# BVE-Reborn/rend3

Hardware: AMD Instinct MI355X
Metric: shaded Mpixels/s @4K (whole frame: cull+compact all cameras, 4 shadow views, PBR opaque, tonemap) (higher is better)
Workload: dtype f32; 1 GPU; BASELINE.json configs[2] stand-in: bistro_like (seed 0xB157, every object owns its geometry), 3840x2160, full PBR opaque + 4 directional shadow views (2048^2), camera dolly, 130 materials with base colour + normal + AO/roughness/metallic maps (RGBA8, mips, trilinear); objects=3000, triangles=2823212, cameras=5, parallelism=single GPU

## Files before the change

bindings/rend3-amd-sys/src/lib.rs:

```rust
#![allow(non_camel_case_types, non_upper_case_globals, clippy::too_many_arguments)]
use std::os::raw::{c_char, c_int, c_void};

pub const R3N_OK: i32 = 0;
pub const R3N_ERR_INVALID_ARG: i32 = -1;
pub const R3N_ERR_HIP: i32 = -2;
pub const R3N_ERR_NO_DEVICE: i32 = -3;
pub const R3N_ERR_STATE: i32 = -4;
pub const R3N_ERR_UNSUPPORTED: i32 = -5;
pub const R3N_ERR_CAPACITY: i32 = -6;
pub const R3N_CAMERA_VIEWPORT: u32 = 0xFFFFFFFF;
pub const R3N_MAX_SHADOW_VIEWS: u32 = 64;
pub const R3N_PASS_DEPTH: u32 = 0;
pub const R3N_PASS_FORWARD: u32 = 1;
pub const R3N_SOURCE_PREDICTED: u32 = 0;
pub const R3N_SOURCE_RESIDUAL: u32 = 1;
pub const R3N_KEY_OPAQUE: u32 = 0;
pub const R3N_KEY_CUTOUT: u32 = 1;
pub const R3N_KEY_BLEND: u32 = 2;
pub const R3N_TEXTURE_RGBA8_UNORM: u32 = 0;
pub const R3N_TEXTURE_RGBA8_UNORM_SRGB: u32 = 1;
pub const R3N_TEXTURE_R8_UNORM: u32 = 2;
pub const R3N_TEXTURE_RG8_UNORM: u32 = 3;
pub const R3N_TEXTURE_BGRA8_UNORM: u32 = 4;
pub const R3N_TEXTURE_BGRA8_UNORM_SRGB: u32 = 5;
// ... 374 lines not shown
}

#[repr(C)]
#[derive(Clone, Copy)]
pub struct r3n_texture_tail_result {
    pub textures: u64,
    pub words_copied: u64,
    pub kernel_launches: u64,
    pub full_syncs: u64,
    pub pool_words_after: u64,
}

#[repr(C)]
#[derive(Clone, Copy)]
pub struct r3n_texture_counters {
    pub update_calls: u64,
    pub kernel_launches: u64,
    pub bytes_staged: u64,
    pub full_syncs: u64,
    pub pool_grows: u64,
    pub pool_words: u64,
    pub live_words: u64,
    pub free_ranges: u64,
}

#[repr(C)]
#[derive(Clone, Copy)]
pub struct r3n_sample_query40 {
    pub id: [u32; 3],
    pub nearest: u32,
    pub u: f32,
    pub v: f32,
    pub ddx: [f32; 2],
    pub ddy: [f32; 2],
}

#[repr(C)]
#[derive(Clone, Copy)]
pub struct r3n_sample_result52 {
    pub rgba: [[f32; 4]; 3],
    pub flags: u32,
}

#[repr(C)]
#[derive(Clone, Copy)]
pub struct r3n_shadow_view272 {
    pub header: r3n_camera_header240,
    pub x: u32,
    pub y: u32,
    pub size: u32,
    pub _pad: [u32; 5],
}

#[repr(C)]
#[derive(Clone, Copy)]
pub struct r3n_frame_desc {
    pub struct_size: u32,
    pub flags: u32,
    pub width: u32,
    pub height: u32,
    pub samples: u32,
    pub shadow_atlas_width: u32,
    pub shadow_atlas_height: u32,
    pub n_shadow_views: u32,
    pub clear_color: [f32; 4],
    pub uniforms: *const r3n_frame_uniforms496,
    pub viewport_header: *const r3n_camera_header240,
    pub shadow_views: *const r3n_shadow_view272,
    pub shadow_view_mask: u64,
    pub directional_buffer: *const c_void,
    pub directional_bytes: u64,
    pub point_buffer: *const c_void,
    pub point_bytes: u64,
    pub skin_inputs: *const r3n_skinning_input40,
    pub n_skeletons: u32,
    pub n_joint_matrices: u32,
    pub joint_matrices: *const f32,
    pub exchange: r3n_exchange_fn,
    pub exchange_user: *mut c_void,
}

#[repr(C)]
#[derive(Clone, Copy)]
pub struct r3n_tri_ref {
    pub object: u32,
    pub triangle: u32,
}

#[repr(C)]
#[derive(Clone, Copy)]
pub struct r3n_host_camera144 {
    pub view: [f32; 16],
    pub projection_kind: u32,
    pub handedness: u32,
    pub aspect_ratio: f32,
    pub _pad: u32,
    pub projection_params: [f32; 16],
}

#[repr(C)]
#[derive(Clone, Copy)]
pub struct r3n_host_directional_light48 {
    pub color: [f32; 3],
    pub intensity: f32,
    pub direction: [f32; 3],
    pub distance: f32,
    pub resolution: u32,
    pub _pad: [u32; 3],
}

#[repr(C)]
#[derive(Clone, Copy)]
pub struct r3n_host_frame {
    pub uniforms: r3n_frame_uniforms496,
    pub viewport_header: r3n_camera_header240,
    pub shadow_atlas_width: u32,
    pub shadow_atlas_height: u32,
    pub n_shadow_views: u32,
    pub _pad0: u32,
    pub camera_location: [f32; 3],
    pub _pad1: f32,
    pub view_proj: [f32; 16],
    pub shadow_views: [r3n_shadow_view272; R3N_MAX_SHADOW_VIEWS as usize],
    pub shadow_handles: [u32; R3N_MAX_SHADOW_VIEWS as usize],
    pub directional_bytes: u64,
    pub directional_buffer: [u8; 8208],
}

#[link(name = "rend3_amd")]
extern "C" {
    pub fn r3n_create(hip_device: c_int, config: *const r3n_config) -> *mut r3n_ctx;
    pub fn r3n_destroy(ctx: *mut r3n_ctx);
    pub fn r3n_last_error(ctx: *const r3n_ctx) -> *const c_char;
    pub fn r3n_create_error() -> *const c_char;
    pub fn r3n_sync(ctx: *mut r3n_ctx) -> c_int;
    pub fn r3n_stream(ctx: *mut r3n_ctx) -> *mut c_void;
    pub fn r3n_mesh_buffer_write(ctx: *mut r3n_ctx, byte_offset: u64, data: *const c_void, bytes: u64) -> c_int;
    pub fn r3n_mesh_blocks_add(ctx: *mut r3n_ctx, blocks: *const r3n_mesh_block24, n: u32, payload: *const c_void, payload_bytes: u64, byte_offsets_out: *mut u64) -> c_int;
    pub fn r3n_mesh_blocks_remove(ctx: *mut r3n_ctx, byte_offsets: *const u64, n: u32) -> c_int;
    pub fn r3n_mesh_compact(ctx: *mut r3n_ctx, opts: *const r3n_mesh_compact_opts, result: *mut r3n_mesh_compact_result, moves_out: *mut r3n_mesh_move24, moves_capacity: u32) -> c_int;
    pub fn r3n_mesh_stats(ctx: *mut r3n_ctx, out: *mut r3n_mesh_counters, reset: c_int) -> c_int;
    pub fn r3n_objects_write(ctx: *mut r3n_ctx, slots: *const u32, records: *const r3n_object128, n: u32, capacity: u32) -> c_int;
    pub fn r3n_materials_write(ctx: *mut r3n_ctx, slots: *const u32, records: *const r3n_material208, keys: *const u8, n: u32) -> c_int;
    pub fn r3n_textures_write(ctx: *mut r3n_ctx, descs: *const r3n_texture_desc32, n_textures: u32, texels: *const u32, n_texels: u64) -> c_int;
    pub fn r3n_textures_write_encoded(ctx: *mut r3n_ctx, descs: *const r3n_texture_desc32, n_textures: u32, payload: *const c_void, payload_bytes: u64) -> c_int;
    pub fn r3n_textures_update(ctx: *mut r3n_ctx, slots: *const u32, descs: *const r3n_texture_desc32, n: u32, payload: *const c_void, payload_bytes: u64) -> c_int;
    pub fn r3n_textures_remove(ctx: *mut r3n_ctx, slots: *const u32, n: u32) -> c_int;
    pub fn r3n_textures_compact(ctx: *mut r3n_ctx, opts: *const r3n_texture_compact_opts, out: *mut r3n_texture_compact_result) -> c_int;
    pub fn r3n_textures_from_texture(ctx: *mut r3n_ctx, items: *const r3n_texture_tail16, n: u32, out: *mut r3n_texture_tail_result) -> c_int;
    pub fn r3n_texture_stats(ctx: *mut r3n_ctx, out: *mut r3n_texture_counters, reset: c_int) -> c_int;
    pub fn r3n_sample_probe(ctx: *mut r3n_ctx, form: u32, queries: *const r3n_sample_query40, n: u32, out: *mut r3n_sample_result52) -> c_int;
    pub fn r3n_texture_cubes_write(ctx: *mut r3n_ctx, descs: *const r3n_texture_desc32, n_cubes: u32, texels: *const u32, n_texels: u64) -> c_int;
    pub fn r3n_skybox_set(ctx: *mut r3n_ctx, cube_id: u32) -> c_int;
    pub fn r3n_blend_order_write(ctx: *mut r3n_ctx, objects_back_to_front: *const u32, n: u32) -> c_int;
    pub fn r3n_blend_objects_write(ctx: *mut r3n_ctx, slots: *const u32, locations: *const f32, n: u32) -> c_int;
    pub fn r3n_blend_sort(ctx: *mut r3n_ctx, camera_location: *const f32) -> c_int;
    pub fn r3n_lights_write(ctx: *mut r3n_ctx, directional_buffer: *const c_void, directional_bytes: u64, point_buffer: *const c_void, point_bytes: u64) -> c_int;
    pub fn r3n_set_output_format(ctx: *mut r3n_ctx, format: u32) -> c_int;
    pub fn r3n_set_skinning_mode(ctx: *mut r3n_ctx, mode: u32) -> c_int;
    pub fn r3n_set_shade_mode(ctx: *mut r3n_ctx, mode: u32) -> c_int;
    pub fn r3n_frame_begin(ctx: *mut r3n_ctx, uniforms: *const r3n_frame_uniforms496, width: u32, height: u32, samples: u32, clear_color: *const f32, shadow_atlas_width: u32, shadow_atlas_height: u32) -> c_int;
    pub fn r3n_skinning(ctx: *mut r3n_ctx, inputs: *const r3n_skinning_input40, n_skeletons: u32, joint_matrices: *const f32, n_joint_matrices: u32) -> c_int;
    pub fn r3n_animation_write(ctx: *mut r3n_ctx, rigs: *const r3n_anim_rig16, n_rigs: u32, joints: *const r3n_anim_joint80, n_joints: u32, clips: *const r3n_anim_clip16, n_clips: u32, tracks: *const r3n_anim_track80, n_tracks: u32, times: *const f32, n_times: u32, values: *const f32, n_values: u32) -> c_int;
    pub fn r3n_pose_skeletons(ctx: *mut r3n_ctx, requests: *const r3n_pose_request16, n: u32) -> c_int;
    pub fn r3n_morph(ctx: *mut r3n_ctx, inputs: *const r3n_morph_input48, n_instances: u32, weights: *const f32, n_weights: u32) -> c_int;
    pub fn r3n_vertex_normals(ctx: *mut r3n_ctx, inputs: *const r3n_normals_input32, n_instances: u32) -> c_int;
    pub fn r3n_vertex_tangents(ctx: *mut r3n_ctx, inputs: *const r3n_tangents_input32, n_instances: u32) -> c_int;
    pub fn r3n_uniform_bake(ctx: *mut r3n_ctx, camera: u32, header: *const r3n_camera_header240) -> c_int;
    pub fn r3n_cull(ctx: *mut r3n_ctx, camera: u32) -> c_int;
    pub fn r3n_hi_z(ctx: *mut r3n_ctx) -> c_int;
    pub fn r3n_shadow_viewport(ctx: *mut r3n_ctx, shadow_camera: u32, x: u32, y: u32, size: u32) -> c_int;
    pub fn r3n_forward(ctx: *mut r3n_ctx, camera: u32, pass: u32, source: u32, material_key: u32) -> c_int;
    pub fn r3n_resolve_opaque(ctx: *mut r3n_ctx) -> c_int;
    pub fn r3n_skybox(ctx: *mut r3n_ctx) -> c_int;
    pub fn r3n_tonemap(ctx: *mut r3n_ctx, host_rgba8: *mut c_void, pitch_bytes: u64) -> c_int;
    pub fn r3n_hdr_write(ctx: *mut r3n_ctx, rgba16f: *const u16, first_pixel: u64, n_pixels: u64) -> c_int;
    pub fn r3n_frame_end(ctx: *mut r3n_ctx) -> c_int;
    pub fn r3n_render_frame(ctx: *mut r3n_ctx, desc: *const r3n_frame_desc) -> c_int;
    pub fn r3n_set_object_range(ctx: *mut r3n_ctx, begin: u32, end: u32) -> c_int;
    pub fn r3n_set_object_owners(ctx: *mut r3n_ctx, owners: *const u8, n: u32, rank: u32) -> c_int;
    pub fn r3n_set_shard_mode(ctx: *mut r3n_ctx, mode: u32) -> c_int;
    pub fn r3n_comm_unique_id(id: *mut u8) -> c_int;
    pub fn r3n_comm_init(ctx: *mut r3n_ctx, ids: *const u8, rank: u32, world: u32) -> c_int;
    pub fn r3n_comm_set_split(ctx: *mut r3n_ctx, mode: u32) -> c_int;
    pub fn r3n_comm_destroy(ctx: *mut r3n_ctx) -> c_int;
    pub fn r3n_set_camera_object_range(ctx: *mut r3n_ctx, camera: u32, begin: u32, end: u32) -> c_int;
    pub fn r3n_exchange_depth(ctx: *mut r3n_ctx, depth_f32: *mut *mut c_void, count: *mut u64) -> c_int;
    pub fn r3n_exchange_buffers(ctx: *mut r3n_ctx, visibility_keys: *mut *mut c_void, visibility_count: *mut u64, shadow_atlas: *mut *mut c_void, shadow_atlas_count: *mut u64) -> c_int;
    pub fn r3n_exchange_shadow_stream(ctx: *mut r3n_ctx, shadow_atlas: *mut *mut c_void, shadow_atlas_count: *mut u64, stream: *mut *mut c_void) -> c_int;
    pub fn r3n_set_row_range(ctx: *mut r3n_ctx, row_begin: u32, row_end: u32) -> c_int;
    pub fn r3n_output_buffer(ctx: *mut r3n_ctx, rgba8: *mut *mut c_void, bytes: *mut u64) -> c_int;
    pub fn r3n_output_buffer_async(ctx: *mut r3n_ctx, rgba8: *mut *mut c_void, bytes: *mut u64, stream: *mut *mut c_void) -> c_int;
    pub fn r3n_output_work_enqueued(ctx: *mut r3n_ctx) -> c_int;
    pub fn r3n_readback_visible_objects(ctx: *mut r3n_ctx, camera: u32, flags: *mut u8, capacity: u32) -> c_int;
    pub fn r3n_readback_triangle_sets(ctx: *mut r3n_ctx, camera: u32, pass: *mut u8, residual: *mut u8, n: u64) -> c_int;
    pub fn r3n_readback_triangle_lists(ctx: *mut r3n_ctx, camera: u32, list: u32, out: *mut r3n_tri_ref, capacity: u64, counts: *mut u32, subcap: *mut u32) -> c_int;
    pub fn r3n_readback_draw_calls(ctx: *mut r3n_ctx, camera: u32, calls: *mut r3n_indirect_call) -> c_int;
    pub fn r3n_readback_raster_stats(ctx: *mut r3n_ctx, big_items: *mut u32) -> c_int;
    pub fn r3n_readback_blend_order(ctx: *mut r3n_ctx, order: *mut u32, rank_base: *mut u32, capacity: u32) -> c_int;
    pub fn r3n_readback_baked(ctx: *mut r3n_ctx, camera: u32, model_view_and_mvp: *mut f32, capacity: u32) -> c_int;
    pub fn r3n_readback_mesh(ctx: *mut r3n_ctx, byte_offset: u64, dst: *mut c_void, bytes: u64) -> c_int;
    pub fn r3n_readback_objects(ctx: *mut r3n_ctx, first_slot: u32, records: *mut r3n_object128, n: u32) -> c_int;
    pub fn r3n_readback_joint_matrices(ctx: *mut r3n_ctx, first_matrix: u32, dst: *mut f32, n_matrices: u32) -> c_int;
    pub fn r3n_readback_texture_descs(ctx: *mut r3n_ctx, descs: *mut r3n_texture_desc32, capacity: u32, n_slots: *mut u32) -> c_int;
    pub fn r3n_readback_texels(ctx: *mut r3n_ctx, first_texel: u64, rgba8: *mut u32, n_texels: u64) -> c_int;
    pub fn r3n_readback_visibility(ctx: *mut r3n_ctx, keys: *mut u64) -> c_int;
    pub fn r3n_readback_depth(ctx: *mut r3n_ctx, depth: *mut f32) -> c_int;
    pub fn r3n_readback_hiz(ctx: *mut r3n_ctx, pyramid: *mut f32, count: u64) -> c_int;
    pub fn r3n_readback_shadow_atlas(ctx: *mut r3n_ctx, atlas: *mut f32) -> c_int;
    pub fn r3n_readback_hdr(ctx: *mut r3n_ctx, rgba16f: *mut u16) -> c_int;
    pub fn r3n_readback_output(ctx: *mut r3n_ctx, rgba8: *mut u8, rgba_f32: *mut f32) -> c_int;
    pub fn r3n_timing_enable(ctx: *mut r3n_ctx, enable: c_int) -> c_int;
    pub fn r3n_timing_overhead(ctx: *mut r3n_ctx, ms_per_span: *mut f64) -> c_int;
    pub fn r3n_set_multi_stream(ctx: *mut r3n_ctx, enable: c_int) -> c_int;
    pub fn r3n_stage_times(ctx: *mut r3n_ctx, ms: *mut f64, launches: *mut u64, reset: c_int) -> c_int;
    pub fn r3n_hbm_copy_rate(ctx: *mut r3n_ctx, bytes: u64, repeats: u32, gb_per_s: *mut f64) -> c_int;
    pub fn r3n_selftest_exact_math(hip_device: c_int, hist: *mut u64, guarded: *mut u64) -> c_int;
    pub fn r3n_selftest_unorm8(hip_device: c_int, n_bad: *mut u32) -> c_int;
    pub fn r3n_host_mat4_mul(a: *const f32, b: *const f32, out: *mut f32);
    pub fn r3n_host_mat4_inverse(m: *const f32, out: *mut f32);
    pub fn r3n_host_look_at(eye: *const f32, center: *const f32, up: *const f32, rh: c_int, out: *mut f32);
    pub fn r3n_host_projection(kind: c_int, params: *const f32, rh: c_int, aspect_ratio: f32, out: *mut f32);
    pub fn r3n_host_frustum_from_matrix(m: *const f32, planes20: *mut f32);
    pub fn r3n_host_frustum_contains_sphere(planes20: *const f32, center: *const f32, radius: f32) -> c_int;
    pub fn r3n_host_bounding_sphere_from_mesh(positions: *const f32, vertex_count: u64, out_center: *mut f32, out_radius: *mut f32);
    pub fn r3n_host_bounding_sphere_apply_transform(center: *const f32, radius: f32, m: *const f32, out_center: *mut f32, out_radius: *mut f32);
    pub fn r3n_host_build_object_records(n: u32, transforms: *const f32, mesh_desc: *const f32, mesh_u32: *const u32, material_index: *const u32, out_records: *mut r3n_object128);
    pub fn r3n_host_calculate_normals(positions: *const f32, vertex_count: u64, indices: *const u32, index_count: u64, left_handed: c_int, normals: *mut f32);
    pub fn r3n_host_calculate_tangents(positions: *const f32, normals: *const f32, uvs: *const f32, vertex_count: u64, indices: *const u32, index_count: u64, tangents: *mut f32);
    pub fn r3n_host_vertex_adjacency(indices: *const u32, index_count: u64, vertex_count: u64, out: *mut u32) -> c_int;
    pub fn r3n_host_shadow_camera(direction: *const f32, distance: f32, resolution: u32, camera_location: *const f32, rh: c_int, out_view: *mut f32, out_proj: *mut f32);
    pub fn r3n_host_allocate_shadow_atlas(handles: *const u32, resolutions: *const u16, n: u32, max_dimension: u32, out_dimensions: *mut u32, out_maps: *mut u32) -> u32;
    pub fn r3n_host_evaluate_frame(camera: *const r3n_host_camera144, lights: *const r3n_host_directional_light48, n_lights: u32, max_atlas_dimension: u32, ambient: *const f32, width: u32, height: u32, samples: u32, object_capacity: u32, out: *mut r3n_host_frame) -> c_int;
}
```

include/r3n.h:

```cpp
#ifndef R3N_H
#define R3N_H

#include <stdint.h>

#ifdef __cplusplus
extern "C" {
#endif

#define R3N_OK 0
#define R3N_ERR_INVALID_ARG (-1)
#define R3N_ERR_HIP (-2)
#define R3N_ERR_NO_DEVICE (-3)
#define R3N_ERR_STATE (-4)
#define R3N_ERR_UNSUPPORTED (-5)
#define R3N_ERR_CAPACITY (-6)

typedef uint32_t r3n_camera;
#define R3N_CAMERA_VIEWPORT 0xFFFFFFFFu
#define R3N_MAX_SHADOW_VIEWS 64u

#define R3N_PASS_DEPTH 0u
#define R3N_PASS_FORWARD 1u
#define R3N_SOURCE_PREDICTED 0u
#define R3N_SOURCE_RESIDUAL 1u
// ... 255 lines not shown
    uint32_t nearest;
    float u, v, ddx[2], ddy[2];
} r3n_sample_query40;
typedef struct r3n_sample_result52 {
    float rgba[3][4];
    uint32_t flags;
} r3n_sample_result52;
int r3n_sample_probe(r3n_ctx *ctx, uint32_t form, const r3n_sample_query40 *queries, uint32_t n, r3n_sample_result52 *out);
int r3n_texture_cubes_write(r3n_ctx *ctx, const r3n_texture_desc32 *descs, uint32_t n_cubes, const uint32_t *texels,
                            uint64_t n_texels);
int r3n_skybox_set(r3n_ctx *ctx, uint32_t cube_id);
int r3n_blend_order_write(r3n_ctx *ctx, const uint32_t *objects_back_to_front, uint32_t n);
int r3n_blend_objects_write(r3n_ctx *ctx, const uint32_t *slots, const float *locations, uint32_t n);
int r3n_blend_sort(r3n_ctx *ctx, const float camera_location[3]);
int r3n_lights_write(r3n_ctx *ctx, const void *directional_buffer, uint64_t directional_bytes,
                     const void *point_buffer, uint64_t point_bytes);

#define R3N_OUTPUT_RGBA8_UNORM_SRGB 0u
#define R3N_OUTPUT_BGRA8_UNORM_SRGB 1u
#define R3N_OUTPUT_RGBA8_UNORM 2u
#define R3N_OUTPUT_BGRA8_UNORM 3u
int r3n_set_output_format(r3n_ctx *ctx, uint32_t format);
#define R3N_SKIN_EXACT 0u
#define R3N_SKIN_MFMA 1u
int r3n_set_skinning_mode(r3n_ctx *ctx, uint32_t mode);
int r3n_set_shade_mode(r3n_ctx *ctx, uint32_t mode);

int r3n_frame_begin(r3n_ctx *ctx, const r3n_frame_uniforms496 *uniforms, uint32_t width, uint32_t height,
                    uint32_t samples, const float clear_color[4], uint32_t shadow_atlas_width,
                    uint32_t shadow_atlas_height);
int r3n_skinning(r3n_ctx *ctx, const r3n_skinning_input40 *inputs, uint32_t n_skeletons, const float *joint_matrices,
                 uint32_t n_joint_matrices);
int r3n_animation_write(r3n_ctx *ctx, const r3n_anim_rig16 *rigs, uint32_t n_rigs, const r3n_anim_joint80 *joints,
                        uint32_t n_joints, const r3n_anim_clip16 *clips, uint32_t n_clips, const r3n_anim_track80 *tracks,
                        uint32_t n_tracks, const float *times, uint32_t n_times, const float *values, uint32_t n_values);
int r3n_pose_skeletons(r3n_ctx *ctx, const r3n_pose_request16 *requests, uint32_t n);
int r3n_morph(r3n_ctx *ctx, const r3n_morph_input48 *inputs, uint32_t n_instances, const float *weights, uint32_t n_weights);
int r3n_vertex_normals(r3n_ctx *ctx, const r3n_normals_input32 *inputs, uint32_t n_instances);
int r3n_vertex_tangents(r3n_ctx *ctx, const r3n_tangents_input32 *inputs, uint32_t n_instances);
int r3n_uniform_bake(r3n_ctx *ctx, r3n_camera camera, const r3n_camera_header240 *header);
int r3n_cull(r3n_ctx *ctx, r3n_camera camera);
int r3n_hi_z(r3n_ctx *ctx);
int r3n_shadow_viewport(r3n_ctx *ctx, r3n_camera shadow_camera, uint32_t x, uint32_t y, uint32_t size);
int r3n_forward(r3n_ctx *ctx, r3n_camera camera, uint32_t pass, uint32_t source, uint32_t material_key);
int r3n_resolve_opaque(r3n_ctx *ctx);
int r3n_skybox(r3n_ctx *ctx);
int r3n_tonemap(r3n_ctx *ctx, void *host_rgba8, uint64_t pitch_bytes);
int r3n_hdr_write(r3n_ctx *ctx, const uint16_t *rgba16f, uint64_t first_pixel, uint64_t n_pixels);
int r3n_frame_end(r3n_ctx *ctx);

typedef struct r3n_shadow_view272 {
    r3n_camera_header240 header;
    uint32_t x, y, size;
    uint32_t _pad[5];
} r3n_shadow_view272;
#define R3N_EXCHANGE_SHADOW 0u
#define R3N_EXCHANGE_PASS1 1u
#define R3N_EXCHANGE_PASS2 2u
typedef int (*r3n_exchange_fn)(void *user, uint32_t site);
#define R3N_FRAME_VIEWPORT_FIRST 1u
#define R3N_FRAME_SHADOW_MASK 2u
typedef struct r3n_frame_desc {
    uint32_t struct_size;
    uint32_t flags;
    uint32_t width, height, samples;
    uint32_t shadow_atlas_width, shadow_atlas_height;
    uint32_t n_shadow_views;
    float clear_color[4];
    const r3n_frame_uniforms496 *uniforms;
    const r3n_camera_header240 *viewport_header;
    const r3n_shadow_view272 *shadow_views;
    uint64_t shadow_view_mask;
    const void *directional_buffer;
    uint64_t directional_bytes;
    const void *point_buffer;
    uint64_t point_bytes;
    const r3n_skinning_input40 *skin_inputs;
    uint32_t n_skeletons, n_joint_matrices;
    const float *joint_matrices;
    r3n_exchange_fn exchange;
    void *exchange_user;
} r3n_frame_desc;
int r3n_render_frame(r3n_ctx *ctx, const r3n_frame_desc *desc);

int r3n_set_object_range(r3n_ctx *ctx, uint32_t begin, uint32_t end);
int r3n_set_object_owners(r3n_ctx *ctx, const uint8_t *owners, uint32_t n, uint32_t rank);
#define R3N_SHARD_OBJECTS 0u
#define R3N_SHARD_ROWS 1u
int r3n_set_shard_mode(r3n_ctx *ctx, uint32_t mode);
#define R3N_COMM_ID_BYTES 128
#define R3N_COMM_IDS 3
int r3n_comm_unique_id(uint8_t *id );
int r3n_comm_init(r3n_ctx *ctx, const uint8_t *ids , uint32_t rank, uint32_t world);
int r3n_comm_set_split(r3n_ctx *ctx, uint32_t mode );
int r3n_comm_destroy(r3n_ctx *ctx);
int r3n_set_camera_object_range(r3n_ctx *ctx, r3n_camera camera, uint32_t begin, uint32_t end);
int r3n_exchange_depth(r3n_ctx *ctx, void **depth_f32, uint64_t *count);
int r3n_exchange_buffers(r3n_ctx *ctx, void **visibility_keys, uint64_t *visibility_count,
                         void **shadow_atlas, uint64_t *shadow_atlas_count);
int r3n_exchange_shadow_stream(r3n_ctx *ctx, void **shadow_atlas, uint64_t *shadow_atlas_count, void **stream);
int r3n_set_row_range(r3n_ctx *ctx, uint32_t row_begin, uint32_t row_end);
int r3n_output_buffer(r3n_ctx *ctx, void **rgba8, uint64_t *bytes);
int r3n_output_buffer_async(r3n_ctx *ctx, void **rgba8, uint64_t *bytes, void **stream);
int r3n_output_work_enqueued(r3n_ctx *ctx);

int r3n_readback_visible_objects(r3n_ctx *ctx, r3n_camera camera, uint8_t *flags, uint32_t capacity);
int r3n_readback_triangle_sets(r3n_ctx *ctx, r3n_camera camera, uint8_t *pass, uint8_t *residual, uint64_t n);
#define R3N_SUBQ 32
typedef struct r3n_tri_ref {
    uint32_t object;
    uint32_t triangle;
} r3n_tri_ref;
int r3n_readback_triangle_lists(r3n_ctx *ctx, r3n_camera camera, uint32_t list, r3n_tri_ref *out, uint64_t capacity,
                                uint32_t counts[3][R3N_SUBQ], uint32_t *subcap);
int r3n_readback_draw_calls(r3n_ctx *ctx, r3n_camera camera, r3n_indirect_call calls[6]);
int r3n_readback_raster_stats(r3n_ctx *ctx, uint32_t big_items[64]);
int r3n_readback_blend_order(r3n_ctx *ctx, uint32_t *order, uint32_t *rank_base, uint32_t capacity);
int r3n_readback_baked(r3n_ctx *ctx, r3n_camera camera, float *model_view_and_mvp, uint32_t capacity);
int r3n_readback_mesh(r3n_ctx *ctx, uint64_t byte_offset, void *dst, uint64_t bytes);
int r3n_readback_objects(r3n_ctx *ctx, uint32_t first_slot, r3n_object128 *records, uint32_t n);
int r3n_readback_joint_matrices(r3n_ctx *ctx, uint32_t first_matrix, float *dst, uint32_t n_matrices);
int r3n_readback_texture_descs(r3n_ctx *ctx, r3n_texture_desc32 *descs, uint32_t capacity, uint32_t *n_slots);
int r3n_readback_texels(r3n_ctx *ctx, uint64_t first_texel, uint32_t *rgba8, uint64_t n_texels);
int r3n_readback_visibility(r3n_ctx *ctx, uint64_t *keys);
int r3n_readback_depth(r3n_ctx *ctx, float *depth);
int r3n_readback_hiz(r3n_ctx *ctx, float *pyramid, uint64_t count);
int r3n_readback_shadow_atlas(r3n_ctx *ctx, float *atlas);
int r3n_readback_hdr(r3n_ctx *ctx, uint16_t *rgba16f);
int r3n_readback_output(r3n_ctx *ctx, uint8_t *rgba8, float *rgba_f32);

#define R3N_STAGE_BAKE 0
#define R3N_STAGE_OBJECT_CULL 1
#define R3N_STAGE_TRIANGLE_CULL 2
#define R3N_STAGE_HIZ 3
#define R3N_STAGE_RASTER 4
#define R3N_STAGE_SHADE 5
#define R3N_STAGE_TONEMAP 6
#define R3N_STAGE_CLEAR 7
#define R3N_STAGE_RASTER_BIG 8
#define R3N_STAGE_SHADOW_RASTER 9
#define R3N_STAGE_SHADOW_RASTER_BIG 10
#define R3N_STAGE_SKINNING 11
#define R3N_STAGE_VERTEX 12
#define R3N_STAGE_POSE 13
#define R3N_STAGE_EXCHANGE_SHADOW 14
#define R3N_STAGE_EXCHANGE_DEPTH 15
#define R3N_STAGE_EXCHANGE_ROWS 16
#define R3N_STAGE_EXCHANGE_KEYS 17
#define R3N_STAGE_RASTER_CUT 18
#define R3N_STAGE_RASTER_BIG_CUT 19
#define R3N_STAGE_SKYBOX 20
#define R3N_STAGE_BLEND_SORT 21
#define R3N_STAGE_MORPH 22
#define R3N_STAGE_NORMALS 23
#define R3N_STAGE_TANGENTS 24
#define R3N_STAGE_COUNT 25
int r3n_timing_enable(r3n_ctx *ctx, int enable);
int r3n_timing_overhead(r3n_ctx *ctx, double *ms_per_span);
int r3n_set_multi_stream(r3n_ctx *ctx, int enable);
int r3n_stage_times(r3n_ctx *ctx, double ms[R3N_STAGE_COUNT], uint64_t launches[R3N_STAGE_COUNT], int reset);
int r3n_hbm_copy_rate(r3n_ctx *ctx, uint64_t bytes, uint32_t repeats, double *gb_per_s);
int r3n_selftest_exact_math(int hip_device, unsigned long long *hist, unsigned long long *guarded);
int r3n_selftest_unorm8(int hip_device, uint32_t *n_bad);

void r3n_host_mat4_mul(const float *a, const float *b, float *out);
void r3n_host_mat4_inverse(const float *m, float *out);
// ... 59 lines not shown
```

rend3_amd/_ffi.py:

```python
import ctypes
import os

import numpy as np

from . import build as _build

vp = ctypes.c_void_p
u32 = ctypes.c_uint32
u64 = ctypes.c_uint64
cint = ctypes.c_int
cfloat = ctypes.c_float

CAMERA_VIEWPORT = 0xFFFFFFFF
PASS_DEPTH, PASS_FORWARD = 0, 1
SOURCE_PREDICTED, SOURCE_RESIDUAL = 0, 1
KEY_OPAQUE, KEY_CUTOUT, KEY_BLEND = 0, 1, 2
STAGES = ["bake", "object_cull", "triangle_cull", "hiz", "raster", "shade", "tonemap", "clear", "raster_big",
          "shadow_raster", "shadow_raster_big", "skinning", "vertex", "pose", "exchange_shadow", "exchange_depth", "exchange_rows", "exchange_keys",
          "raster_cut", "raster_big_cut", "skybox", "blend_sort"]
STAGE_NAMES = STAGES + ["morph", "normals"]
STAGE_TABLE = STAGE_NAMES + ["tangents"]

COMM_ID_BYTES, COMM_IDS = 128, 3

SIGNATURES = {
    "r3n_create": (vp, [cint, vp]),
    "r3n_destroy": (None, [vp]),
    "r3n_last_error": (ctypes.c_char_p, [vp]),
    "r3n_create_error": (ctypes.c_char_p, []),
    "r3n_sync": (cint, [vp]),
    "r3n_stream": (vp, [vp]),
    "r3n_mesh_buffer_write": (cint, [vp, u64, vp, u64]),
    "r3n_mesh_blocks_add": (cint, [vp, vp, u32, vp, u64, vp]),
    "r3n_mesh_blocks_remove": (cint, [vp, vp, u32]),
    "r3n_mesh_compact": (cint, [vp, vp, vp, vp, u32]),
    "r3n_mesh_stats": (cint, [vp, vp, cint]),
    "r3n_objects_write": (cint, [vp, vp, vp, u32, u32]),
    "r3n_materials_write": (cint, [vp, vp, vp, vp, u32]),
    "r3n_textures_write": (cint, [vp, vp, u32, vp, u64]),
    "r3n_textures_write_encoded": (cint, [vp, vp, u32, vp, u64]),
    "r3n_textures_update": (cint, [vp, vp, vp, u32, vp, u64]),
    "r3n_textures_remove": (cint, [vp, vp, u32]),
    "r3n_textures_compact": (cint, [vp, vp, vp]),
    "r3n_textures_from_texture": (cint, [vp, vp, u32, vp]),
    "r3n_texture_stats": (cint, [vp, vp, cint]),
    "r3n_sample_probe": (cint, [vp, u32, vp, u32, vp]),
    "r3n_texture_cubes_write": (cint, [vp, vp, u32, vp, u64]),
    "r3n_skybox_set": (cint, [vp, u32]),
    "r3n_animation_write": (cint, [vp, vp, u32, vp, u32, vp, u32, vp, u32, vp, u32, vp, u32]),
    "r3n_pose_skeletons": (cint, [vp, vp, u32]),
    "r3n_morph": (cint, [vp, vp, u32, vp, u32]),
    "r3n_vertex_normals": (cint, [vp, vp, u32]),
    "r3n_vertex_tangents": (cint, [vp, vp, u32]),
    "r3n_set_output_format": (cint, [vp, u32]),
    "r3n_set_shade_mode": (cint, [vp, u32]),
    "r3n_set_skinning_mode": (cint, [vp, u32]),
    "r3n_blend_order_write": (cint, [vp, vp, u32]),
    "r3n_blend_objects_write": (cint, [vp, vp, vp, u32]),
    "r3n_blend_sort": (cint, [vp, vp]),
    "r3n_lights_write": (cint, [vp, vp, u64, vp, u64]),
    "r3n_frame_begin": (cint, [vp, vp, u32, u32, u32, vp, u32, u32]),
    "r3n_skinning": (cint, [vp, vp, u32, vp, u32]),
    "r3n_uniform_bake": (cint, [vp, u32, vp]),
    "r3n_cull": (cint, [vp, u32]),
    "r3n_hi_z": (cint, [vp]),
    "r3n_shadow_viewport": (cint, [vp, u32, u32, u32, u32]),
    "r3n_forward": (cint, [vp, u32, u32, u32, u32]),
    "r3n_resolve_opaque": (cint, [vp]),
    "r3n_skybox": (cint, [vp]),
    "r3n_tonemap": (cint, [vp, vp, u64]),
    "r3n_hdr_write": (cint, [vp, vp, u64, u64]),
    "r3n_frame_end": (cint, [vp]),
    "r3n_render_frame": (cint, [vp, vp]),
    "r3n_set_object_range": (cint, [vp, u32, u32]),
    "r3n_set_object_owners": (cint, [vp, vp, u32, u32]),
    "r3n_exchange_buffers": (cint, [vp, vp, vp, vp, vp]),
    "r3n_exchange_shadow_stream": (cint, [vp, vp, vp, vp]),
    "r3n_set_shard_mode": (cint, [vp, u32]),
    "r3n_comm_unique_id": (cint, [vp]),
    "r3n_comm_init": (cint, [vp, vp, u32, u32]),
    "r3n_comm_destroy": (cint, [vp]),
    "r3n_comm_set_split": (cint, [vp, u32]),
    "r3n_timing_overhead": (cint, [vp, vp]),
    "r3n_set_camera_object_range": (cint, [vp, u32, u32, u32]),
    "r3n_exchange_depth": (cint, [vp, vp, vp]),
    "r3n_set_row_range": (cint, [vp, u32, u32]),
    "r3n_output_buffer": (cint, [vp, vp, vp]),
    "r3n_output_buffer_async": (cint, [vp, vp, vp, vp]),
    "r3n_output_work_enqueued": (cint, [vp]),
    "r3n_readback_visible_objects": (cint, [vp, u32, vp, u32]),
    "r3n_readback_triangle_sets": (cint, [vp, u32, vp, vp, u64]),
    "r3n_readback_triangle_lists": (cint, [vp, u32, u32, vp, u64, vp, vp]),
    "r3n_readback_draw_calls": (cint, [vp, u32, vp]),
    "r3n_readback_raster_stats": (cint, [vp, vp]),
    "r3n_readback_blend_order": (cint, [vp, vp, vp, u32]),
    "r3n_readback_baked": (cint, [vp, u32, vp, u32]),
    "r3n_readback_mesh": (cint, [vp, u64, vp, u64]),
    "r3n_readback_objects": (cint, [vp, u32, vp, u32]),
    "r3n_readback_texture_descs": (cint, [vp, vp, u32, vp]),
    "r3n_readback_texels": (cint, [vp, u64, vp, u64]),
    "r3n_readback_joint_matrices": (cint, [vp, u32, vp, u32]),
    "r3n_readback_visibility": (cint, [vp, vp]),
    "r3n_readback_depth": (cint, [vp, vp]),
    "r3n_readback_hiz": (cint, [vp, vp, u64]),
    "r3n_readback_shadow_atlas": (cint, [vp, vp]),
    "r3n_readback_hdr": (cint, [vp, vp]),
    "r3n_readback_output": (cint, [vp, vp, vp]),
    "r3n_timing_enable": (cint, [vp, cint]),
    "r3n_stage_times": (cint, [vp, vp, vp, cint]),
    "r3n_set_multi_stream": (cint, [vp, cint]),
    "r3n_hbm_copy_rate": (cint, [vp, u64, u32, vp]),
    "r3n_selftest_exact_math": (cint, [cint, vp, vp]),
    "r3n_selftest_unorm8": (cint, [cint, vp]),
    "r3n_host_mat4_mul": (None, [vp, vp, vp]),
    "r3n_host_mat4_inverse": (None, [vp, vp]),
    "r3n_host_look_at": (None, [vp, vp, vp, cint, vp]),
    "r3n_host_projection": (None, [cint, vp, cint, cfloat, vp]),
    "r3n_host_frustum_from_matrix": (None, [vp, vp]),
    "r3n_host_frustum_contains_sphere": (cint, [vp, vp, cfloat]),
    "r3n_host_bounding_sphere_from_mesh": (None, [vp, u64, vp, vp]),
    "r3n_host_bounding_sphere_apply_transform": (None, [vp, cfloat, vp, vp, vp]),
    "r3n_host_build_object_records": (None, [u32, vp, vp, vp, vp, vp]),
    "r3n_host_calculate_normals": (None, [vp, u64, vp, u64, cint, vp]),
    "r3n_host_calculate_tangents": (None, [vp, vp, vp, u64, vp, u64, vp]),
    "r3n_host_vertex_adjacency": (cint, [vp, u64, u64, vp]),
    "r3n_host_shadow_camera": (None, [vp, cfloat, u32, vp, cint, vp, vp]),
    "r3n_host_allocate_shadow_atlas": (u32, [vp, vp, u32, u32, vp, vp]),
    "r3n_host_evaluate_frame": (cint, [vp, vp, u32, u32, vp, u32, u32, u32, u32, vp]),
}

MAX_SHADOW_VIEWS = 64
MAX_MORPH_TARGETS = 256
EXCHANGE_SITES = ("shadow", "pass1", "pass2")
FRAME_VIEWPORT_FIRST, FRAME_SHADOW_MASK = 1, 2
EXCHANGE_FN = ctypes.CFUNCTYPE(cint, vp, u32)


class ShadowView272(ctypes.Structure):
    _fields_ = [("header", ctypes.c_uint8 * 240), ("x", u32), ("y", u32), ("size", u32), ("_pad", u32 * 5)]


class HostCamera144(ctypes.Structure):
    _fields_ = [("view", cfloat * 16), ("projection_kind", u32), ("handedness", u32), ("aspect_ratio", cfloat), ("_pad", u32),
                ("projection_params", cfloat * 16)]


class HostFrame(ctypes.Structure):
    _fields_ = [("uniforms", ctypes.c_uint8 * 496), ("viewport_header", ctypes.c_uint8 * 240),
                ("shadow_atlas_width", u32), ("shadow_atlas_height", u32), ("n_shadow_views", u32), ("_pad0", u32),
                ("camera_location", cfloat * 3), ("_pad1", cfloat), ("view_proj", cfloat * 16),
                ("shadow_views", ShadowView272 * MAX_SHADOW_VIEWS), ("shadow_handles", u32 * MAX_SHADOW_VIEWS),
                ("directional_bytes", u64), ("directional_buffer", ctypes.c_uint8 * (16 + 128 * MAX_SHADOW_VIEWS))]


class FrameDesc(ctypes.Structure):
    _fields_ = [("struct_size", u32), ("flags", u32), ("width", u32), ("height", u32), ("samples", u32),
                ("shadow_atlas_width", u32), ("shadow_atlas_height", u32), ("n_shadow_views", u32), ("clear_color", cfloat * 4),
                ("uniforms", vp), ("viewport_header", vp), ("shadow_views", vp), ("shadow_view_mask", u64),
                ("directional_buffer", vp), ("directional_bytes", u64), ("point_buffer", vp), ("point_bytes", u64),
                ("skin_inputs", vp), ("n_skeletons", u32), ("n_joint_matrices", u32), ("joint_matrices", vp),
                ("exchange", EXCHANGE_FN), ("exchange_user", vp)]


class TextureCounters(ctypes.Structure):
    _fields_ = [(name, u64) for name in ("update_calls", "kernel_launches", "bytes_staged", "full_syncs", "pool_grows", "pool_words",
                                         "live_words", "free_ranges")]


class TextureCompactOpts(ctypes.Structure):
    _fields_ = [("max_words", u64), ("stage_words", u64)]


class TextureCompactResult(ctypes.Structure):
    _fields_ = [(name, u64) for name in ("textures_moved", "words_moved", "passes", "kernel_launches", "full_syncs", "pool_words_before",
                                         "pool_words_after", "free_ranges_after")]


MESH_BLOCK_ZERO = 1


class MeshBlock24(ctypes.Structure):
    _fields_ = [("payload_offset", u64), ("words", u64), ("flags", u32), ("_pad", u32)]


class MeshMove24(ctypes.Structure):
    _fields_ = [("old_byte_offset", u64), ("new_byte_offset", u64), ("padded_words", u64)]


class MeshCompactOpts(ctypes.Structure):
    _fields_ = [("max_words", u64), ("stage_words", u64)]


class MeshCompactResult(ctypes.Structure):
    _fields_ = [(name, u64) for name in ("blocks_moved", "words_moved", "passes", "kernel_launches", "full_syncs", "pool_words_before",
                                         "pool_words_after", "free_ranges_after", "relocate_ns")]


class MeshCounters(ctypes.Structure):
    _fields_ = [(name, u64) for name in ("add_calls", "remove_calls", "compact_calls", "bytes_staged", "launches", "full_waits", "growths",
                                         "blocks_live", "live_words", "pool_words", "free_ranges", "buffer_words")]


class TextureTail16(ctypes.Structure):
    _fields_ = [("dst_slot", u32), ("src_slot", u32), ("start_mip", u32), ("mip_count", u32)]


class TextureTailResult(ctypes.Structure):
    _fields_ = [(name, u64) for name in ("textures", "words_copied", "kernel_launches", "full_syncs", "pool_words_after")]


class Config(ctypes.Structure):
    _fields_ = [("struct_size", u32), ("max_big_items", u32), ("shade_mode", u32), ("_pad", u32), ("reserved", u64 * 2)]


assert ctypes.sizeof(ShadowView272) == 272 and ctypes.sizeof(HostCamera144) == 144 and ctypes.sizeof(FrameDesc) == 152
assert ctypes.sizeof(HostFrame) == 26712 and ctypes.sizeof(Config) == 32
assert ctypes.sizeof(MeshBlock24) == 24 and ctypes.sizeof(MeshMove24) == 24 and ctypes.sizeof(MeshCounters) == 96

_LIB = None


def library_path():
    return _build.SO


def lib():
    global _LIB
    if _LIB is None:
        try:
            import torch
        except ImportError:
            pass
        path = os.environ.get("R3N_LIB") or _build.build()
        if not os.path.exists(path):
            raise RuntimeError("librend3_amd.so is missing and could not be built; the HIP path has no fallback")
        l = ctypes.CDLL(path)
        for name, (res, args) in SIGNATURES.items():
            fn = getattr(l, name)
            fn.restype = res
            fn.argtypes = args
        _LIB = l
    return _LIB


def ptr(a):
    if a is None:
        return None
    assert isinstance(a, np.ndarray) and a.flags["C_CONTIGUOUS"], "need a contiguous ndarray"
    return a.ctypes.data_as(vp)


ERR_CAPACITY = -6


class R3nError(RuntimeError):
    def __init__(self, message, code=None):
        super().__init__(message)
        self.code = code


def check(ctx, code, what):
    if code != 0:
        msg = lib().r3n_last_error(ctx)
        raise R3nError(f"{what} failed ({code}): {msg.decode() if msg else ''}", code)
```

rend3_amd/csrc/device_math.h:

```cpp
#pragma once
#include <hip/hip_runtime.h>

#include "exact_math.h"
#include "layouts.h"

#define R3N_DEV __device__ __forceinline__

typedef uint32_t r3n_u32x4 __attribute__((ext_vector_type(4)));
typedef uint32_t r3n_u32x16 __attribute__((ext_vector_type(16)));
template <class V> R3N_DEV V scalar_load(const void *p) {
    const unsigned long long v = (unsigned long long)p;
    const uint32_t lo = (uint32_t)__builtin_amdgcn_readfirstlane((uint32_t)v), hi = (uint32_t)__builtin_amdgcn_readfirstlane((uint32_t)(v >> 32));
    const unsigned long long u = ((unsigned long long)hi << 32) | (unsigned long long)lo;
    return *reinterpret_cast<__attribute__((address_space(4))) const V *>(u);
}

R3N_DEV void mul_vec4(const float *__restrict__ m, float x, float y, float z, float w, float o[4]) {
#pragma unroll
    for (int r = 0; r < 4; ++r) o[r] = ((m[r] * x + m[4 + r] * y) + m[8 + r] * z) + m[12 + r] * w;
}
R3N_DEV void mul_point(const float *__restrict__ m, const float v[3], float o[4]) { mul_vec4(m, v[0], v[1], v[2], 1.0f, o); }

typedef float f2 __attribute__((ext_vector_type(2)));
R3N_DEV f2 splat2(float v) { return (f2){v, v}; }
// ... 18 lines not shown
    static R3N_DEV float sqrt(float x) { return __builtin_amdgcn_sqrtf(x); }
    static R3N_DEV float rsqrt(float x) { return __builtin_amdgcn_rsqf(x); }
};

R3N_DEV float dot3(const float a[3], const float b[3]) { return (a[0] * b[0] + a[1] * b[1]) + a[2] * b[2]; }
template <class M> R3N_DEV float dot3m(const float a[3], const float b[3]) { return M::mad(a[2], b[2], M::mad(a[1], b[1], a[0] * b[0])); }
template <class M> R3N_DEV void normalize3m(float v[3]) {
    const float r = M::rsqrt(dot3m<M>(v, v));
    v[0] *= r; v[1] *= r; v[2] *= r;
}
template <class M> R3N_DEV void mul_vec4m(const float *__restrict__ m, float x, float y, float z, float w, float o[4]) {
#pragma unroll
    for (int r = 0; r < 4; r += 2) {
        const f2 c0 = {m[r], m[r + 1]}, c1 = {m[4 + r], m[5 + r]}, c2 = {m[8 + r], m[9 + r]}, c3 = {m[12 + r], m[13 + r]};
        const f2 t = M::mad(c3, splat2(w), M::mad(c2, splat2(z), M::mad(c1, splat2(y), c0 * splat2(x))));
        o[r] = t.x; o[r + 1] = t.y;
    }
}
template <class M> R3N_DEV void mat3_mul_vec3m(const float *__restrict__ c0, const float *__restrict__ c1, const float *__restrict__ c2,
                                               const float v[3], float o[3]) {
    const f2 t = M::mad((f2){c2[0], c2[1]}, splat2(v[2]), M::mad((f2){c1[0], c1[1]}, splat2(v[1]), (f2){c0[0], c0[1]} * splat2(v[0])));
    o[0] = t.x; o[1] = t.y;
    o[2] = M::mad(c2[2], v[2], M::mad(c1[2], v[1], c0[2] * v[0]));
}
R3N_DEV float sat(float v) { return fminf(fmaxf(v, 0.0f), 1.0f); }
R3N_DEV void normalize3(float v[3]) {
    float r = 1.0f / sqrtf(dot3(v, v));
    v[0] *= r; v[1] *= r; v[2] *= r;
}
R3N_DEV void mat3_mul_vec3(const float *__restrict__ c0, const float *__restrict__ c1, const float *__restrict__ c2,
                           const float v[3], float o[3]) {
#pragma unroll
    for (int r = 0; r < 3; ++r) o[r] = (c0[r] * v[0] + c1[r] * v[1]) + c2[r] * v[2];
}

R3N_DEV float det3_xyw(const float p0[4], const float p1[4], const float p2[4]) {
    float ax = p0[0], ay = p0[1], az = p0[3];
    float bx = p1[0], by = p1[1], bz = p1[3];
    float cx = p2[0], cy = p2[1], cz = p2[3];
    return (ax * (by * cz - cy * bz) - bx * (ay * cz - cy * az)) + cx * (ay * bz - by * az);
}

R3N_DEV uint32_t ceil_log2_ge1(float x) {
    x = fmaxf(x, 1.0f);
    uint32_t b = __float_as_uint(x);
    uint32_t e = (b >> 23) & 0xFFu;
    if (e == 0xFFu) return 1000u;
    uint32_t l = e - 127u;
    return (b & 0x7FFFFFu) ? l + 1u : l;
}

R3N_DEV uint32_t clamp_texel(float v, uint32_t dim) {
    if (!(v >= 0.0f)) return 0u;
    float top = (float)(dim - 1u);
    if (v >= top) return dim - 1u;
    return (uint32_t)v;
}

R3N_DEV uint32_t mip_dim(uint32_t d, uint32_t k) {
    uint32_t v = d >> k;
    return v ? v : 1u;
}

struct __attribute__((packed, aligned(4))) r3n_words2 { uint32_t x, y; };
struct __attribute__((packed, aligned(4))) r3n_words3 { uint32_t x, y, z; };
struct __attribute__((packed, aligned(4))) r3n_words4 { uint32_t x, y, z, w; };
R3N_DEV void fetch_vec3(const uint32_t *__restrict__ mesh, uint32_t byte_off, uint32_t vtx, float o[3]) {
    const uint32_t w = byte_off / 4u + vtx * 3u;
    const r3n_words3 v = *reinterpret_cast<const r3n_words3 *>(mesh + w);
    o[0] = __uint_as_float(v.x);
    o[1] = __uint_as_float(v.y);
    o[2] = __uint_as_float(v.z);
}
R3N_DEV void fetch_indices3(const uint32_t *__restrict__ mesh, uint32_t first, uint32_t idx[3]) {
    const r3n_words3 v = *reinterpret_cast<const r3n_words3 *>(mesh + first);
    idx[0] = v.x; idx[1] = v.y; idx[2] = v.z;
}

struct TriSetup {
    float e[3][3];
    float z[3];
    float det;
    bool valid;
};

R3N_DEV void setup_triangle(const float p[3][4], float half_w, float half_h, bool positive_visible, TriSetup &ts) {
    float h[3][3], zc[3];
#pragma unroll
    for (int k = 0; k < 3; ++k) {
        h[k][0] = (p[k][0] + p[k][3]) * half_w;
        h[k][1] = (p[k][3] - p[k][1]) * half_h;
        h[k][2] = p[k][3];
        zc[k] = p[k][2];
    }
#pragma unroll
    for (int i = 0; i < 3; ++i) {
        const float *a = h[(i + 1) % 3], *b = h[(i + 2) % 3];
        ts.e[i][0] = a[1] * b[2] - a[2] * b[1];
        ts.e[i][1] = a[2] * b[0] - a[0] * b[2];
        ts.e[i][2] = a[0] * b[1] - a[1] * b[0];
    }
    float det = (h[0][0] * ts.e[0][0] + h[0][1] * ts.e[0][1]) + h[0][2] * ts.e[0][2];
    ts.valid = positive_visible ? (det < 0.0f) : (det > 0.0f);
    if (det < 0.0f) {
        det = -det;
#pragma unroll
        for (int i = 0; i < 3; ++i)
#pragma unroll
            for (int c = 0; c < 3; ++c) ts.e[i][c] = -ts.e[i][c];
    }
    ts.det = det;
    bool planar = false;
    if (h[0][2] > 0.0f && h[1][2] > 0.0f && h[2][2] > 0.0f) {
        float sx[3], sy[3], zn[3];
#pragma unroll
        for (int k = 0; k < 3; ++k) {
            const float rw = exact_math::rcp(h[k][2]);
            sx[k] = h[k][0] * rw; sy[k] = h[k][1] * rw; zn[k] = zc[k] * rw;
        }
        const float ax = sx[1] - sx[0], ay = sy[1] - sy[0], bx = sx[2] - sx[0], by = sy[2] - sy[0];
        const float az = zn[1] - zn[0], bz = zn[2] - zn[0];
        const float ia = exact_math::rcp(ax * by - bx * ay);
        const float gx = (az * by - bz * ay) * ia, gy = (bz * ax - az * bx) * ia;
        const float c = (zn[0] - gx * sx[0]) - gy * sy[0];
        if (gx - gx == 0.0f && gy - gy == 0.0f && c - c == 0.0f) {
            ts.z[0] = gx; ts.z[1] = gy; ts.z[2] = c;
            planar = true;
        }
    }
    if (!planar) {
        ts.z[0] = ((ts.e[0][0] * zc[0] + ts.e[1][0] * zc[1]) + ts.e[2][0] * zc[2]) / det;
        ts.z[1] = ((ts.e[0][1] * zc[0] + ts.e[1][1] * zc[1]) + ts.e[2][1] * zc[2]) / det;
        ts.z[2] = ((ts.e[0][2] * zc[0] + ts.e[1][2] * zc[1]) + ts.e[2][2] * zc[2]) / det;
    }
}

R3N_DEV bool f32_positive(float a) { return (int)__float_as_uint(a) > 0; }
R3N_DEV float edge_threshold(float A, float B) {
    return (A > 0.0f || (A == 0.0f && B > 0.0f)) ? 0.0f : 1.401298464324817e-45f;
}
R3N_DEV bool edge_eval_thr(const TriSetup &ts, const float thr[3], float px, float py, float E[3]) {
    bool in = true;
#pragma unroll
    for (int i = 0; i < 3; ++i) {
        const float v = (ts.e[i][0] * px + ts.e[i][1] * py) + ts.e[i][2];
        E[i] = v;
        in = in && (v >= thr[i]);
    }
    return in;
}
R3N_DEV bool edge_eval(const TriSetup &ts, float px, float py, float E[3]) {
    bool in = true;
#pragma unroll
    for (int i = 0; i < 3; ++i) {
        const float A = ts.e[i][0], B = ts.e[i][1];
        const float v = (A * px + B * py) + ts.e[i][2];
        E[i] = v;
        const float thr = edge_threshold(A, B);
        in = in && (v >= thr);
    }
    return in;
}

R3N_DEV float frag_depth(const TriSetup &ts, float px, float py) { return (ts.z[0] * px + ts.z[1] * py) + ts.z[2]; }
R3N_DEV bool tri_bounds(const float p[3][4], float half_w, float half_h, int vw, int vh, int &x0, int &y0, int &x1,
                        int &y1) {
    float mnx = INFINITY, mny = INFINITY, mxx = -INFINITY, mxy = -INFINITY;
    bool ok = true;
    bool any = false;
    auto add = [&](float x, float y, float w) {
        if (!(w > 1e-30f)) { ok = false; return; }
        const float sx = (x / w + 1.0f) * half_w;
        const float sy = (1.0f - y / w) * half_h;
        if (!(sx - sx == 0.0f) || !(sy - sy == 0.0f)) { ok = false; return; }
        mnx = fminf(mnx, sx); mxx = fmaxf(mxx, sx);
        mny = fminf(mny, sy); mxy = fmaxf(mxy, sy);
        any = true;
    };
    const bool all_front = p[0][3] > 0.0f && p[1][3] > 0.0f && p[2][3] > 0.0f;
    if (all_front) {
#pragma unroll
        for (int k = 0; k < 3; ++k) add(p[k][0], p[k][1], p[k][3]);
    } else {
        float dA[3], dB[3];
        bool crossA = false, crossB = false;
#pragma unroll
        for (int k = 0; k < 3; ++k) {
            dA[k] = p[k][2];
            dB[k] = p[k][3] - p[k][2];
            crossA = crossA || !(dA[k] >= 0.0f);
            crossB = crossB || !(dB[k] >= 0.0f);
        }
        if (crossA && crossB) {
            ok = false;
        } else if (!crossA && !crossB) {
            ok = false;
        } else {
            const float *d = crossA ? dA : dB;
#pragma unroll
            for (int k = 0; k < 3; ++k) {
                const int n = (k + 1) % 3;
                if (d[k] >= 0.0f) add(p[k][0], p[k][1], p[k][3]);
                if ((d[k] >= 0.0f) != (d[n] >= 0.0f)) {
                    const float t = d[k] / (d[k] - d[n]);
                    add(p[k][0] + t * (p[n][0] - p[k][0]), p[k][1] + t * (p[n][1] - p[k][1]),
                        p[k][3] + t * (p[n][3] - p[k][3]));
                }
            }
            if (ok && !any) return false;
        }
    }
    if (!ok) {
// ... 12 lines not shown
```

rend3_amd/csrc/kernels_raster.h:

```cpp
#pragma once
#include "device_math.h"
#include "texture.h"

struct RasterArgs {
    const r3n_camera_header240 *hdr;
    const r3n_object128 *objects;
    const uint32_t *mesh;
    const r3n_baked128 *baked;
    const r3n_material208 *materials;
    const uint8_t *material_keys;
    uint32_t n_materials;
    const uint32_t *tri_base;
    const r3n_tri_ref8 *list;
    const uint32_t *sub_counts;
    uint32_t subcap;
    uint32_t key;
    uint32_t vp_x, vp_y, vp_w, vp_h;
    uint32_t target_pitch;
    unsigned long long *vis;
    uint32_t *depth;
    r3n_big_item *big_items;
    uint32_t *big_count;
    uint32_t big_capacity;
    r3n_big_uv *big_uv;
    TextureArgs tex;
    unsigned long long *frag_keys;
    uint32_t *frag_vals;
    uint32_t *frag_count;
    uint32_t frag_capacity;
    uint32_t *frag_head;
    uint32_t *status;
    uint32_t row_begin, row_end;
};

R3N_DEV float cutout_alpha(uint32_t mat_flags, float mat_alpha, float tex_alpha, float vertex_alpha) {
    float alpha = 1.0f;
    if (mat_flags & R3N_FLAGS_ALBEDO_ACTIVE) {
        alpha = tex_alpha;
        if (mat_flags & R3N_FLAGS_ALBEDO_BLEND) alpha *= vertex_alpha;
    }
    alpha *= mat_alpha;
    return alpha;
}

R3N_DEV float fetch_color_alpha(const r3n_object128 &ob, const uint32_t *__restrict__ mesh, uint32_t vtx) {
    const uint32_t off = ob.vertex_attribute_start_offsets[5];
    if (off == R3N_INVALID) return 1.0f;
    const uint32_t w = mesh[off / 4u + vtx];
    return (float)((w >> 24) & 0xFFu) / 255.0f;
}

struct TriWork {
    TriSetup ts;
    float va[3];
    uint32_t material;
    uint32_t mat_flags;
    float mat_alpha, mat_cutoff;
    uint32_t slot1;
    float uv[3][2];
    bool alpha_tex;
    uint32_t tex0;
    bool nearest;
    float uvt[12];
    r3n_texture_desc32 tdesc;
    bool cutout;
    float thr[3];
    int x0, y0, x1, y1;
};


template <bool DEPTH_ONLY, bool TEX, bool NOCUT = false>
R3N_DEV bool prepare_triangle(const RasterArgs &a, uint32_t obj, uint32_t tri, bool positive_visible, TriWork &tw) {
    const r3n_object128 &ob = a.objects[obj];
    const uint4 of = *reinterpret_cast<const uint4 *>(reinterpret_cast<const char *>(&ob) + offsetof(r3n_object128, first_index));
    const uint32_t enabled = ob.enabled;
    asm volatile("" : : "v"(of.x), "v"(of.w), "v"(enabled));
    if (enabled == 0u) return false;
    const uint32_t first = of.x + tri * 3u;
    const uint32_t pos_off = of.w;
    uint32_t idx[3];
    float p[3][4];
    fetch_indices3(a.mesh, first, idx);
#pragma unroll
    for (int k = 0; k < 3; ++k) {
        float v[3];
        fetch_vec3(a.mesh, pos_off, idx[k], v);
        mul_point(a.baked[obj].model_view_proj, v, p[k]);
    }
    const float half_w = (float)a.vp_w / 2.0f, half_h = (float)a.vp_h / 2.0f;
    setup_triangle(p, half_w, half_h, positive_visible, tw.ts);
    if (!tw.ts.valid) return false;
    if (!tri_bounds(p, half_w, half_h, (int)a.vp_w, (int)a.vp_h, tw.x0, tw.y0, tw.x1, tw.y1)) return false;
    tw.y0 = max(tw.y0, (int)a.row_begin);
    tw.y1 = min(tw.y1, (int)min(a.row_end, a.vp_h) - 1);
    if (tw.y0 > tw.y1) return false;
#pragma unroll
    for (int i = 0; i < 3; ++i) tw.thr[i] = edge_threshold(tw.ts.e[i][0], tw.ts.e[i][1]);
    tw.cutout = !NOCUT && a.key == R3N_KEY_CUTOUT;
    tw.material = of.z < a.n_materials ? of.z : 0u;
    tw.va[0] = tw.va[1] = tw.va[2] = 1.0f;
    tw.mat_flags = 0u; tw.mat_alpha = 1.0f; tw.mat_cutoff = 0.0f;
    tw.alpha_tex = false;
#pragma unroll
    for (int k = 0; k < 3; ++k) tw.uv[k][0] = tw.uv[k][1] = 0.0f;
    if (tw.cutout) {
#pragma unroll
        for (int k = 0; k < 3; ++k) tw.va[k] = fetch_color_alpha(ob, a.mesh, idx[k]);
        const r3n_material208 &m = a.materials[tw.material];
        tw.mat_flags = m.flags; tw.mat_alpha = m.albedo[3]; tw.mat_cutoff = m.alpha_cutout;
        tw.alpha_tex = TEX && (m.flags & R3N_FLAGS_ALBEDO_ACTIVE) && m.textures[0] != 0u;
        if (TEX && tw.alpha_tex) {
#pragma unroll
            for (int k = 0; k < 3; ++k) fetch_uv0(a.mesh, ob.vertex_attribute_start_offsets[3], idx[k], tw.uv[k]);
        }
    }
    if (!DEPTH_ONLY) tw.slot1 = a.tri_base[obj] + tri + 1u;
    return true;
}

#define R3N_PREREAD_SMALL 0
#define R3N_PREREAD_MS 1
#define R3N_PREREAD_VIEWPORT 0
#define R3N_PREREAD_BIG 0
template <bool DEPTH_ONLY, bool TEX, bool HOIST = false, bool SHORTA = false>
R3N_DEV float cutout_texture_alpha(const RasterArgs &a, const TriWork &tw, int x, int y) {
    if (!TEX || !tw.alpha_tex) return 1.0f;
    float coords[2], ddx[2], ddy[2];
    if (HOIST) {
        if (DEPTH_ONLY) {
            frag_coords(tw.ts, tw.uv, nullptr, x, y, coords, ddx, ddy);
            return tex_sample_alpha<MathExact, SHORTA>(a.tex, tw.tex0, tw.tdesc, false, coords[0], coords[1], ddx, ddx);
        }
        frag_coords(tw.ts, tw.uv, tw.uvt, x, y, coords, ddx, ddy);
        return tex_sample_alpha<MathExact, SHORTA>(a.tex, tw.tex0, tw.tdesc, tw.nearest, coords[0], coords[1], ddx, ddy);
    }
    const r3n_material208 &m = a.materials[tw.material];
    const uint32_t id = m.textures[0];
    r3n_texture_desc32 d{};
    if (id - 1u < a.tex.count) d = a.tex.descs[id - 1u];
    if (DEPTH_ONLY) {
        frag_coords(tw.ts, tw.uv, nullptr, x, y, coords, ddx, ddy);
        return tex_sample_alpha<MathExact, SHORTA>(a.tex, id, d, false, coords[0], coords[1], ddx, ddx);
    }
    frag_coords(tw.ts, tw.uv, m.uv_transform0, x, y, coords, ddx, ddy);
    return tex_sample_alpha<MathExact, SHORTA>(a.tex, id, d, (m.flags & R3N_FLAGS_NEAREST) != 0u, coords[0], coords[1], ddx, ddy);
}

__device__ static const float k_sample_pos4[4][2] = {{0.375f, 0.125f}, {0.875f, 0.375f}, {0.125f, 0.625f}, {0.625f, 0.875f}};

R3N_DEV void global_max_u32(uint32_t *p, uint32_t v) {
    typedef __attribute__((address_space(1))) uint32_t *gp_t;
    (void)__hip_atomic_fetch_max((gp_t)(unsigned long long)p, v, __ATOMIC_RELAXED, __HIP_MEMORY_SCOPE_AGENT);
}
R3N_DEV uint32_t global_add_u32(uint32_t *p, uint32_t v) {
    typedef __attribute__((address_space(1))) uint32_t *gp_t;
    return __hip_atomic_fetch_add((gp_t)(unsigned long long)p, v, __ATOMIC_RELAXED, __HIP_MEMORY_SCOPE_AGENT);
}
R3N_DEV void global_max_u64(unsigned long long *p, unsigned long long v) {
    typedef __attribute__((address_space(1))) unsigned long long *gp_t;
    (void)__hip_atomic_fetch_max((gp_t)(unsigned long long)p, v, __ATOMIC_RELAXED, __HIP_MEMORY_SCOPE_AGENT);
}
R3N_DEV void global_max_u32_at(uint32_t *base, uint32_t byte_off, uint32_t v) {
    typedef __attribute__((address_space(1))) uint32_t *gp_t;
    typedef __attribute__((address_space(1))) char *gc_t;
    (void)__hip_atomic_fetch_max((gp_t)((gc_t)(unsigned long long)base + byte_off), v, __ATOMIC_RELAXED, __HIP_MEMORY_SCOPE_AGENT);
}
R3N_DEV void global_max_u64_at(unsigned long long *base, uint32_t byte_off, unsigned long long v) {
    typedef __attribute__((address_space(1))) unsigned long long *gp_t;
    typedef __attribute__((address_space(1))) char *gc_t;
    (void)__hip_atomic_fetch_max((gp_t)((gc_t)(unsigned long long)base + byte_off), v, __ATOMIC_RELAXED, __HIP_MEMORY_SCOPE_AGENT);
}

template <bool DEPTH_ONLY>
R3N_DEV uint32_t target_pixel(const RasterArgs &a, uint32_t x, uint32_t y) {
    return __umul24(a.vp_y + y, a.target_pitch) + (a.vp_x + x);
}

template <bool DEPTH_ONLY, bool PREREAD, int S = 1, bool TEX = false, bool BLEND = false, bool HOIST = false, bool SHORTA = false>
// ... 86 lines not shown
        for (int sm = 0; sm < S; ++sm)
            if (mask & (1u << sm))
                global_max_u64(&a.vis[pix + (size_t)sm], ((unsigned long long)__float_as_uint(zs[sm]) << 32) | (unsigned long long)tw.slot1);
    }
}

template <bool DEPTH_ONLY, bool FINE>
R3N_DEV void shade_pixel_cmpx(const RasterArgs &a, const TriWork &tw, int x, int y, uint32_t b, int rx0, int rx1, int ry1) {
    float E[3];
#pragma unroll
    for (int i = 0; i < 3; ++i) E[i] = (tw.ts.e[i][0] * ((float)x + 0.5f) + tw.ts.e[i][1] * ((float)y + 0.5f)) + tw.ts.e[i][2];
    const float z = frag_depth(tw.ts, (float)x + 0.5f, (float)y + 0.5f);
    const uint32_t zb = __float_as_uint(z) & 0x7FFFFFFFu;
    const uint32_t pix = target_pixel<DEPTH_ONLY>(a, (uint32_t)x, (uint32_t)y);
    unsigned long long save;
    typedef __attribute__((address_space(1))) void *gv_t;
#define R3N_CMPX_CHAIN                                                                                             \
    "s_mov_b64 %[save], exec\n\t"                                                                                   \
    "v_cmpx_le_i32 vcc, %[rx0], %[x]\n\tv_cmpx_ge_i32 vcc, %[rx1], %[x]\n\tv_cmpx_ge_i32 vcc, %[ry1], %[y]\n\t"                                        \
    "v_cmpx_le_f32 vcc, %[t0], %[e0]\n\tv_cmpx_le_f32 vcc, %[t1], %[e1]\n\tv_cmpx_le_f32 vcc, %[t2], %[e2]\n\t"     \
    "v_cmpx_le_f32 vcc, 0, %[z]\n\tv_cmpx_ge_f32 vcc, 1.0, %[z]\n\t"
    if (DEPTH_ONLY) {
        if (FINE)
            asm volatile("s_mov_b64 %[save], exec\n\tv_cmpx_gt_u32 vcc, 64, %[b]\n\t"
                         "v_cmpx_le_i32 vcc, %[rx0], %[x]\n\tv_cmpx_ge_i32 vcc, %[rx1], %[x]\n\tv_cmpx_ge_i32 vcc, %[ry1], %[y]\n\t"
                         "v_cmpx_le_f32 vcc, %[t0], %[e0]\n\tv_cmpx_le_f32 vcc, %[t1], %[e1]\n\tv_cmpx_le_f32 vcc, %[t2], %[e2]\n\t"
                         "v_cmpx_le_f32 vcc, 0, %[z]\n\tv_cmpx_ge_f32 vcc, 1.0, %[z]\n\t"
                         "global_atomic_umax %[off], %[data], %[base]\n\t"
                         "s_mov_b64 exec, %[save]"
                         : [save] "=&s"(save)
                         : [b] "v"(b), [rx0] "s"(rx0), [rx1] "s"(rx1), [x] "v"(x), [ry1] "s"(ry1), [y] "v"(y), [t0] "s"(tw.thr[0]), [e0] "v"(E[0]),
                           [t1] "s"(tw.thr[1]), [e1] "v"(E[1]), [t2] "s"(tw.thr[2]), [e2] "v"(E[2]), [z] "v"(z), [off] "v"(pix << 2),
                           [data] "v"(zb), [base] "s"((gv_t)(unsigned long long)a.depth)
                         : "vcc", "memory");
        else
            asm volatile(R3N_CMPX_CHAIN
                         "global_atomic_umax %[off], %[data], %[base]\n\t"
                         "s_mov_b64 exec, %[save]"
                         : [save] "=&s"(save)
                         : [rx0] "s"(rx0), [rx1] "s"(rx1), [x] "v"(x), [ry1] "s"(ry1), [y] "v"(y), [t0] "s"(tw.thr[0]), [e0] "v"(E[0]),
                           [t1] "s"(tw.thr[1]), [e1] "v"(E[1]), [t2] "s"(tw.thr[2]), [e2] "v"(E[2]), [z] "v"(z), [off] "v"(pix << 2),
                           [data] "v"(zb), [base] "s"((gv_t)(unsigned long long)a.depth)
                         : "vcc", "memory");
    } else {
        const unsigned long long key = ((unsigned long long)zb << 32) | (unsigned long long)tw.slot1;
        if (FINE)
            asm volatile("s_mov_b64 %[save], exec\n\tv_cmpx_gt_u32 vcc, 64, %[b]\n\t"
                         "v_cmpx_le_i32 vcc, %[rx0], %[x]\n\tv_cmpx_ge_i32 vcc, %[rx1], %[x]\n\tv_cmpx_ge_i32 vcc, %[ry1], %[y]\n\t"
                         "v_cmpx_le_f32 vcc, %[t0], %[e0]\n\tv_cmpx_le_f32 vcc, %[t1], %[e1]\n\tv_cmpx_le_f32 vcc, %[t2], %[e2]\n\t"
                         "v_cmpx_le_f32 vcc, 0, %[z]\n\tv_cmpx_ge_f32 vcc, 1.0, %[z]\n\t"
                         "global_atomic_umax_x2 %[off], %[data], %[base]\n\t"
                         "s_mov_b64 exec, %[save]"
                         : [save] "=&s"(save)
                         : [b] "v"(b), [rx0] "s"(rx0), [rx1] "s"(rx1), [x] "v"(x), [ry1] "s"(ry1), [y] "v"(y), [t0] "s"(tw.thr[0]), [e0] "v"(E[0]),
                           [t1] "s"(tw.thr[1]), [e1] "v"(E[1]), [t2] "s"(tw.thr[2]), [e2] "v"(E[2]), [z] "v"(z), [off] "v"(pix << 3),
                           [data] "v"(key), [base] "s"((gv_t)(unsigned long long)a.vis)
                         : "vcc", "memory");
        else
            asm volatile(R3N_CMPX_CHAIN
                         "global_atomic_umax_x2 %[off], %[data], %[base]\n\t"
                         "s_mov_b64 exec, %[save]"
                         : [save] "=&s"(save)
                         : [rx0] "s"(rx0), [rx1] "s"(rx1), [x] "v"(x), [ry1] "s"(ry1), [y] "v"(y), [t0] "s"(tw.thr[0]), [e0] "v"(E[0]),
                           [t1] "s"(tw.thr[1]), [e1] "v"(E[1]), [t2] "s"(tw.thr[2]), [e2] "v"(E[2]), [z] "v"(z), [off] "v"(pix << 3),
                           [data] "v"(key), [base] "s"((gv_t)(unsigned long long)a.vis)
                         : "vcc", "memory");
    }
#undef R3N_CMPX_CHAIN
}

#define R3N_BIG_THR_SHIFT 29u
#define R3N_BIG_MATERIAL_MASK 0x1FFFFFFFu
R3N_DEV uint32_t pack_thresholds(const float thr[3]) {
    return ((thr[0] != 0.0f ? 1u : 0u) | (thr[1] != 0.0f ? 2u : 0u) | (thr[2] != 0.0f ? 4u : 0u)) << R3N_BIG_THR_SHIFT;
}

#define R3N_SMALL_MAX 8
#define R3N_TILE 32
#define R3N_SMALL_OCC 1
#define R3N_ITEM_ALIGN 16
#define R3N_FINE_LW_DEPTH 3
#define R3N_FINE_LW_VIS 3

template <bool DEPTH_ONLY, int S = 1, bool TEX = false, bool NOCUT = false, bool SHORTA = false>
R3N_DEV void raster_small_body(const RasterArgs &a) {
    const uint32_t q = blockIdx.x % R3N_SUBQ;
    const uint32_t n = a.sub_counts[a.key * R3N_SUBQ + q];
    const r3n_tri_ref8 *list = a.list + (size_t)(a.key * R3N_SUBQ + q) * a.subcap;
    const uint32_t bq = __builtin_amdgcn_readfirstlane((blockIdx.x * (blockDim.x >> 6) + (threadIdx.x >> 6)) % R3N_BIGQ);
    const bool positive_visible = (a.hdr->flags & R3N_PCU_POSITIVE_AREA_VISIBLE) != 0u;
    const uint32_t stride = (gridDim.x / R3N_SUBQ) * blockDim.x;
    for (uint32_t i = (blockIdx.x / R3N_SUBQ) * blockDim.x + threadIdx.x; i < n; i += stride) {
        const r3n_tri_ref8 ref = list[i];
        TriWork tw;
        if (!prepare_triangle<DEPTH_ONLY, TEX, NOCUT>(a, ref.object, ref.triangle, positive_visible, tw)) continue;
        const int bw = tw.x1 - tw.x0 + 1, bh = tw.y1 - tw.y0 + 1;
        if (bw <= R3N_SMALL_MAX && bh <= R3N_SMALL_MAX) {
            for (int y = tw.y0; y <= tw.y1; ++y)
                for (int x = tw.x0; x <= tw.x1; ++x) shade_pixel<DEPTH_ONLY, R3N_PREREAD_SMALL != 0, S, TEX, false, false, SHORTA>(a, tw, x, y);
        } else {
            const int ax0 = tw.x0 & ~(R3N_ITEM_ALIGN - 1);
            const uint32_t tx = (uint32_t)(tw.x1 - ax0 + R3N_TILE) / R3N_TILE, ty = (uint32_t)(bh + (R3N_TILE - 1)) / R3N_TILE;
            const uint32_t cnt = tx * ty;
            const uint32_t start = global_add_u32(&a.big_count[bq], cnt);
            r3n_big_item *big = a.big_items + (size_t)bq * a.big_capacity;
            for (uint32_t t = 0; t < cnt; ++t) {
                const uint32_t ix = t % tx, iy = t / tx;
                const int rx0 = max(ax0 + (int)ix * R3N_TILE, tw.x0), ry0 = tw.y0 + (int)iy * R3N_TILE;
                const int rx1 = min(ax0 + (int)ix * R3N_TILE + (R3N_TILE - 1), tw.x1), ry1 = min(ry0 + (R3N_TILE - 1), tw.y1);
                if (start + t < a.big_capacity) {
                    r3n_big_item it;
#pragma unroll
                    for (int i = 0; i < 3; ++i) {
#pragma unroll
                        for (int c = 0; c < 3; ++c) it.e[i][c] = tw.ts.e[i][c];
                        it.z[i] = tw.ts.z[i];
                    }
                    it.slot1 = DEPTH_ONLY ? 0u : tw.slot1;
                    it.material = tw.material | pack_thresholds(tw.thr);
                    it.xy0 = (uint32_t)rx0 | ((uint32_t)ry0 << 16);
                    it.xy1 = (uint32_t)rx1 | ((uint32_t)ry1 << 16);
                    big[start + t] = it;
                    if (tw.cutout) {
                        r3n_big_uv bu;
#pragma unroll
                        for (int k = 0; k < 3; ++k) { bu.uv[k][0] = tw.uv[k][0]; bu.uv[k][1] = tw.uv[k][1]; bu.va[k] = tw.va[k]; }
                        bu._pad[0] = bu._pad[1] = bu._pad[2] = 0u;
                        a.big_uv[(size_t)bq * a.big_capacity + start + t] = bu;
                    }
                } else {
                    for (int y = ry0; y <= ry1; ++y)
                        for (int x = rx0; x <= rx1; ++x) shade_pixel<DEPTH_ONLY, R3N_PREREAD_SMALL != 0, S, TEX, false, false, SHORTA>(a, tw, x, y);
                }
            }
        }
    }
}

template <bool DEPTH_ONLY, int S = 1, bool TEX = false, bool NOCUT = false, bool SHORTA = false>
__global__ __launch_bounds__(256, R3N_SMALL_OCC) void k_raster_small(RasterArgs a) {
    raster_small_body<DEPTH_ONLY, S, TEX, NOCUT, SHORTA>(a);
}
struct BlendSetupArgs {
    const uint32_t *order;
    const uint32_t *rank_base;
    uint32_t n_objects;
    const unsigned long long *mask;
    const uint32_t *slot_base;
};
__global__ __launch_bounds__(256) void k_blend_setup(RasterArgs a, BlendSetupArgs b) {
    const uint32_t total = b.rank_base[b.n_objects];
    const uint32_t g = blockIdx.x * 256u + threadIdx.x;
    if (g >= total) return;
    uint32_t lo = 0, hi = b.n_objects;
    while (hi - lo > 1u) {
        const uint32_t mid = (lo + hi) >> 1;
        if (b.rank_base[mid] <= g) lo = mid; else hi = mid;
    }
    const uint32_t obj = b.order[lo], tri = g - b.rank_base[lo];
    const uint32_t sb = b.slot_base[obj];
    if (sb == R3N_INVALID) return;
    const uint32_t bit = sb + tri;
    if (!((b.mask[bit >> 6] >> (bit & 63u)) & 1ull)) return;
    const bool positive_visible = (a.hdr->flags & R3N_PCU_POSITIVE_AREA_VISIBLE) != 0u;
    TriWork tw;
    if (!prepare_triangle<false, false>(a, obj, tri, positive_visible, tw)) return;
    const int bw = tw.x1 - tw.x0 + 1, bh = tw.y1 - tw.y0 + 1;
    const uint32_t tx = (uint32_t)(bw + (R3N_TILE - 1)) / R3N_TILE, ty = (uint32_t)(bh + (R3N_TILE - 1)) / R3N_TILE;
    const uint32_t cnt = tx * ty;
    const uint32_t bq = (blockIdx.x * 4u + (threadIdx.x >> 6)) % R3N_BIGQ;
    const uint32_t start = atomicAdd(&a.big_count[bq], cnt);
    r3n_big_item *big = a.big_items + (size_t)bq * a.big_capacity;
    for (uint32_t t = 0; t < cnt; ++t) {
        const uint32_t ix = t % tx, iy = t / tx;
        const int rx0 = tw.x0 + (int)ix * R3N_TILE, ry0 = tw.y0 + (int)iy * R3N_TILE;
        const int rx1 = min(rx0 + (R3N_TILE - 1), tw.x1), ry1 = min(ry0 + (R3N_TILE - 1), tw.y1);
        if (start + t >= a.big_capacity) {
            __hip_atomic_store(a.status, 1u, __ATOMIC_RELAXED, __HIP_MEMORY_SCOPE_SYSTEM);
            continue;
        }
        r3n_big_item it;
#pragma unroll
        for (int i = 0; i < 3; ++i) {
#pragma unroll
            for (int c = 0; c < 3; ++c) it.e[i][c] = tw.ts.e[i][c];
            it.z[i] = tw.ts.z[i];
        }
        it.slot1 = tw.slot1;
        it.material = g | pack_thresholds(tw.thr);
        it.xy0 = (uint32_t)rx0 | ((uint32_t)ry0 << 16);
        it.xy1 = (uint32_t)rx1 | ((uint32_t)ry1 << 16);
        big[start + t] = it;
    }
}

template <int S = 8, bool MS = false, int SH = S>
R3N_DEV bool block_may_cover(const TriSetup &ts, int bx, int by, int rx1, int ry1) {
    const float lo = MS ? 0.125f : 0.5f, hi = MS ? 0.875f : 0.5f;
    const float x_lo = (float)bx + lo, x_hi = (float)min(bx + (S - 1), rx1) + hi;
    const float y_lo = (float)by + lo, y_hi = (float)min(by + (SH - 1), ry1) + hi;
    bool may = true;
#pragma unroll
    for (int i = 0; i < 3; ++i) {
        const float A = ts.e[i][0], B = ts.e[i][1];
        const float px = f32_positive(A) ? x_hi : x_lo, py = f32_positive(B) ? y_hi : y_lo;
        const float v = (A * px + B * py) + ts.e[i][2];
        may = may && !(v < 0.0f);
    }
    return may;
}

R3N_DEV void unpack_thresholds(uint32_t mt, float thr[3]) {
#pragma unroll
    for (int i = 0; i < 3; ++i) thr[i] = __uint_as_float((mt >> (R3N_BIG_THR_SHIFT + (uint32_t)i)) & 1u);
}

template <bool DEPTH_ONLY, int S, bool TEX, bool BLEND, bool SHORTA>
R3N_DEV void scan_work_item(const RasterArgs &a, const TriWork &w, uint32_t kxy0, uint32_t kxy1, uint32_t lane) {
    const int lx = (int)(lane & 7u), ly = (int)(lane >> 3);
    const int rx0 = (int)(kxy0 & 0xFFFFu), ry0 = (int)(kxy0 >> 16);
    const int rx1 = (int)(kxy1 & 0xFFFFu), ry1 = (int)(kxy1 >> 16);
    const int gx0 = rx0 & ~(R3N_ITEM_ALIGN - 1);
    if (rx1 - gx0 < 32 && ry1 - ry0 < 32) {
        constexpr int LW = DEPTH_ONLY ? R3N_FINE_LW_DEPTH : R3N_FINE_LW_VIS, FW = 1 << LW, FH = 16 >> LW, LC = 5 - LW;
// ... 338 lines not shown
```

rend3_amd/csrc/r3n.hip:

```cpp
#include <fcntl.h>
#include <hip/hip_runtime.h>
#include <time.h>
#include <unistd.h>

#include <algorithm>
#include <atomic>
#include <cstdio>
#include <cstdlib>
#include <cstring>
#include <map>
#include <string>
#include <vector>

#include "comm.h"
#include "hip_owned.h"
#include "kernels_cull.h"
#include "kernels_raster.h"
#define R3N_SHADE_DECL_ONLY
#include "kernels_shade.h"
#include "skybox.h"
#include "blend_sort.h"
#include "mesh_reloc.h"
#include "morph.h"
#include "normals.h"
#include "tangents.h"
#include "texel_alloc.h"
#include "texel_compact.h"
#include "texel_tail.h"
#include "texture_jobs.h"
#include "vertex_block.h"

namespace {

using hip_owned::DeviceBuffer;
using hip_owned::DeviceSpan;
using hip_owned::Event;
using hip_owned::PinnedHost;
using hip_owned::Stream;

struct CamState {
    r3n_camera_header240 hdr{};
    bool has_hdr = false;
    bool has_prev = false;
    bool culled = false;
    int cur = 0;
    int last = -1;
    uint32_t vp_x = 0, vp_y = 0, vp_size = 0;
    DeviceSpan d_hdr;
    DeviceBuffer own_hdr;
    uint64_t hdr_frame = ~0ull;
    uint64_t baked_frame = ~0ull;
    DeviceBuffer chain;
    uint32_t chain_epoch = 0;
    uint64_t object_pass_frame = ~0ull;
    DeviceBuffer baked, vis_flags, vis_list, block_sums, block_off;
    DeviceBuffer first_entry;
    DeviceBuffer slot_base[2], mask[2], predicted[2], sub_counts[2], counts[2];
    uint32_t subcap[2] = {0, 0};
    uint64_t key_objects[2][3] = {};
    DeviceBuffer residual;
    bool range_set = false;
    uint32_t range_begin = 0, range_end = 0xFFFFFFFFu;
    uint32_t band_begin = 0, band_end = 0xFFFFFFFFu;
};

std::string g_create_error;

}

#define R3N_AUX_STREAMS 2

#define R3N_BIG_GRID 8192
#define R3N_SMALL_GRID 2048
#define R3N_BIG_LDS 40960
#define R3N_SMALL_LDS 24576
#define R3N_VIEWPORT_BIG_LDS 49152
#define R3N_QLANES R3N_AUX_STREAMS
static_assert(R3N_AUX_STREAMS >= 1, "the shadow views draw on auxiliary streams");

struct r3n_ctx {
    int device = 0;
    Stream stream;
    Stream aux[R3N_AUX_STREAMS];
    Event fork_ev[R3N_AUX_STREAMS];
    Stream shade;
    Event vp_ev, shade_done[2];
    bool shade_pending[2] = {false, false};
    bool shade_unjoined = false;
    int shade_last = 0;
    int slot = 0;
    uint64_t frame_no = 0;
    bool overlap = true;
    bool always_fork = false;
    bool resolve_classes = true;
    bool fused_frame = false;
    DeviceBuffer alt_vis, alt_atlas, alt_vp_baked;
    static constexpr size_t kFbUniforms = 0, kFbViewportHdr = 512, kFbDir = 768, kFbShadowHdr = 3072,
                            kFbPoint = kFbShadowHdr + 256 * R3N_MAX_SHADOW_VIEWS, kFbBytes = kFbPoint + 8448;
    static constexpr int kFbHost = 4;
    DeviceBuffer fb_dev[2];
    PinnedHost fb_host[kFbHost];
    Event fb_ev[kFbHost];
    bool fb_pending[kFbHost] = {};
    uint64_t main_epoch = 1, lane_epoch[R3N_AUX_STREAMS] = {};
    DeviceBuffer big_count_all;
    static constexpr size_t kBigCountWords = (size_t)(1 + R3N_QLANES) * 64 * R3N_BIGQ;
    bool exchanged_this_frame = false;
    std::vector<uint8_t> h_dir, h_point;
    uint64_t lights_version = 1, slot_lights_version[2] = {0, 0};
    Event join_ev[R3N_AUX_STREAMS];
    bool aux_used[R3N_AUX_STREAMS] = {};
    bool multi_stream = true;
    std::string err;
    DeviceBuffer mesh, objects, materials, material_keys;
    DeviceSpan dir_buf, point_buf, fu;
    DeviceBuffer spheres, obj_meta;
    bool meta_dirty = false;
    uint32_t capacity = 0, n_materials = 0;
    std::vector<uint32_t> h_ntri;
    std::vector<uint32_t> h_material;
    std::vector<uint8_t> h_material_key;
    std::vector<r3n_material208> h_materials;
    std::vector<uint8_t> h_tex_short;
    DeviceBuffer material_feat;
    DeviceBuffer view_lights[2];
    uint32_t resolve_variants = 0;
    bool classes_dirty = true;
    struct Tune {
        uint32_t big_lds = R3N_BIG_LDS, vp_big_lds = R3N_VIEWPORT_BIG_LDS;
        uint32_t small_lds = R3N_SMALL_LDS, vp_small_lds = 0;
        uint32_t cut_big_lds = 0, vp_cut_big_lds = 0, cut_small_lds = 0, vp_cut_small_lds = 0;
        uint32_t prio_main = 1, prio_shade = 1, prio_aux = 1;
        uint32_t timed_pipeline = 0;
        uint32_t cull_lds = 0, vp_cull_lds = 0;
        uint32_t resolve_lds = 0;
        uint32_t big_grid = R3N_BIG_GRID, small_grid = R3N_SMALL_GRID;
        uint32_t comm_serial = 1;
    } tune;
    bool cutout_short_dirty = true, cutout_short = false;
    bool key_census_dirty = true;
    uint64_t key_objects[3] = {0, 0, 0};
    uint64_t total_tris = 0;
    bool tri_base_dirty = true;
    DeviceBuffer tri_base, slot_table;
    DeviceBuffer skin_inputs, skin_matrices, skin_wave_skeleton, skin_wave_first, skin_joint_counts;
    uint32_t skinning_mode = R3N_SKIN_EXACT, skin_max_joints = 0;
    std::vector<r3n_skinning_input40> h_skin_inputs;
    uint32_t skin_total_waves = 0;
    DeviceBuffer morph_block;
    DeviceBuffer normals_block;
    DeviceBuffer tangents_block;
    uint32_t slot_table_size = 0;
    CamState canon;
    uint32_t width = 0, height = 0, samples = 1, atlas_w = 0, atlas_h = 0;
    float clear[4] = {0, 0, 0, 0};
    bool in_frame = false;
    bool blended_this_frame = false;
    bool resolved_this_frame = false;
    DeviceBuffer vis, hdr16, out8, out_f32, atlas, hiz;
    r3n_hiz_desc hizd{};
    bool hiz_plane_ready = false;
    DeviceBuffer tri_rec, alt_tri_rec, tri_seen;
    DeviceBuffer blend_order, blend_rank_base, frag_keys, frag_vals, frag_count, frag_head, samples16;
    PinnedHost status_host;
    uint32_t *status_dev = nullptr;
    std::vector<uint32_t> h_blend_order;
    uint32_t n_blend = 0, blend_tris = 0;
    DeviceBuffer blend_set_slots, blend_set_locations, blend_sort_scratch;
    bool blend_sorted = false;
    uint32_t frag_capacity = 32u << 20;
    DeviceBuffer tex_descs, tex_texels, tex_level_off, srgb8_decode;
    uint32_t n_textures = 0;
    uint64_t n_texels = 0;
    texel_alloc::Pool tex_alloc;
    std::vector<r3n_texture_desc32> h_tex_descs;
    std::vector<uint64_t> h_tex_words;
    std::vector<uint8_t> h_tex_live;
    std::vector<uint8_t> h_tex_hot;
    uint64_t sync_serial = 0, tex_sync_seen = 0;
    DeviceBuffer tex_stage, tex_jobs;
    std::vector<DeviceBuffer> tex_retired;
    Stream tex_stream;
    r3n_texture_counters tex_stats{};
    texel_alloc::Pool mesh_alloc;
    std::map<uint64_t, uint64_t> mesh_blocks;
    bool mesh_pooled = false;
    bool mesh_appended = false;
    uint64_t mesh_sync_seen = 0;
    r3n_mesh_counters mesh_stats{};
    Event mesh_reloc_ev[2];
    struct Cube { size_t first_word; uint32_t n, srgb; };
    DeviceBuffer cube_texels;
    std::vector<Cube> cubes;
    uint32_t sky_cube = 0;
    bool sky_window = false;
    bool resolve_on_shade = false;
    uint32_t sky_samples_form = R3N_SKY_SAMPLES_ALL;
    DeviceBuffer edge_list, edge_count;
    uint32_t edge_capacity_override = 0;
    DeviceBuffer anim_rigs, anim_joints, anim_clips, anim_tracks, anim_times, anim_values, pose_requests;
    std::vector<r3n_anim_rig16> h_anim_rigs;
    std::vector<r3n_anim_clip16> h_anim_clips;
    uint32_t n_pose_requests = 0, pose_matrix_end = 0, anim_max_joints = 1;
    DeviceBuffer big_uv[1 + R3N_QLANES];
    DeviceBuffer srgb_thr;
    DeviceBuffer srgb_lut;
    uint32_t output_format = R3N_OUTPUT_RGBA8_UNORM_SRGB;
    uint32_t shade_mode = R3N_SHADE_EXACT;
    DeviceBuffer big_items[1 + R3N_QLANES];
    DeviceSpan big_count[1 + R3N_QLANES];
    uint32_t forward_index_lane[1 + R3N_QLANES] = {};
    uint32_t big_capacity = (2u << 20) / R3N_BIGQ;
    CamState viewport;
    std::map<uint32_t, CamState> shadows;
    uint32_t range_begin = 0, range_end = 0xFFFFFFFFu;
    uint32_t row_begin = 0, row_end = 0xFFFFFFFFu;
    bool shard_rows = false;
    struct Comm {
        bool on = false;
        bool by_objects = false;
// ... 366 lines not shown
    HIP_WAIT(c, hipStreamSynchronize(c->stream));
    TRY(run_object_pass(c, c->canon, 0, ObjOwn{0u, 0u, nullptr, 0u}, c->tri_base.as<uint32_t>(), c->stream));
    c->slot_table_size = (uint32_t)(c->total_tris >> R3N_SLOT_TABLE_SHIFT) + 1u;
    TRY(ensure(c, c->slot_table, (size_t)c->slot_table_size * 4u, false, -1));
    hipLaunchKernelGGL(k_build_slot_table, dim3((c->slot_table_size + 255u) / 256u), dim3(256), 0, c->stream,
                       c->tri_base.as<uint32_t>(), c->capacity, c->slot_table.as<uint32_t>(), c->slot_table_size);
    TRY(check_launch(c, "k_build_slot_table"));
    c->tri_base_dirty = false;
    return R3N_OK;
}

void build_hiz_desc(r3n_hiz_desc &d, uint32_t w, uint32_t h) {
    d.width = w; d.height = h;
    uint32_t m = std::max(w, h), n = 0;
    while (m) { ++n; m >>= 1; }
    d.mips = std::min<uint32_t>(n, R3N_MAX_HIZ_MIPS);
    uint32_t off = 0;
    for (uint32_t k = 0; k < R3N_MAX_HIZ_MIPS; ++k) {
        d.offset[k] = off;
        if (k < d.mips) off += std::max(1u, w >> k) * std::max(1u, h >> k);
    }
}
size_t hiz_elements(const r3n_hiz_desc &d) {
    size_t n = 0;
    for (uint32_t k = 0; k < d.mips; ++k) n += (size_t)std::max(1u, d.width >> k) * std::max(1u, d.height >> k);
    return n;
}

void recycle_spans(r3n_ctx *c) {
    for (auto &s : c->spans) {
        c->event_pool.push_back(std::move(s.a));
        c->event_pool.push_back(std::move(s.b));
    }
    c->spans.clear();
}

int drain_timing(r3n_ctx *c) {
    if (c->spans.empty()) return R3N_OK;
    TRY(sync_all(c));
    for (auto &s : c->spans) {
        float ms = 0.f;
        if (hipEventElapsedTime(&ms, s.a, s.b) == hipSuccess) c->stage_ms[s.stage] += std::max(0.0, (double)ms - c->span_overhead_ms);
    }
    recycle_spans(c);
    return R3N_OK;
}

int read_timeline(r3n_ctx *c, float *out, int max) {
    if (c->spans.empty()) return 0;
    if (sync_all(c) != R3N_OK) return -1;
    std::vector<hipStream_t> streams;
    int n = 0;
    for (auto &s : c->spans) {
        float t0 = 0.f, t1 = 0.f;
        size_t si = std::find(streams.begin(), streams.end(), s.stream) - streams.begin();
        if (si == streams.size()) streams.push_back(s.stream);
        if (n < max && hipEventElapsedTime(&t0, c->spans[0].a, s.a) == hipSuccess && hipEventElapsedTime(&t1, c->spans[0].a, s.b) == hipSuccess) {
            out[4 * n + 0] = (float)s.stage; out[4 * n + 1] = (float)si; out[4 * n + 2] = t0; out[4 * n + 3] = t1;
            ++n;
        }
    }
    recycle_spans(c);
    return n;
}

int apply_tuning(r3n_ctx *c, const char *kv) {
    r3n_ctx::Tune t = c->tune;
    std::string text(kv ? kv : "");
    for (size_t at = 0; at < text.size();) {
        while (at < text.size() && (text[at] == ' ' || text[at] == ',')) ++at;
        if (at >= text.size()) break;
        const size_t end = text.find_first_of(" ,", at), eq = text.find('=', at);
        if (eq == std::string::npos || (end != std::string::npos && eq > end)) return fail(c, R3N_ERR_INVALID_ARG, "tuning: expected key=value");
        const std::string key = text.substr(at, eq - at);
        char *stop = nullptr;
        const unsigned long val = std::strtoul(text.c_str() + eq + 1, &stop, 10);
        if (stop == text.c_str() + eq + 1 || (*stop && *stop != ' ' && *stop != ',')) return fail(c, R3N_ERR_INVALID_ARG, "tuning: " + key + " wants an unsigned number");
        struct { const char *name; uint32_t *p; unsigned long lo, hi, step; } keys[] = {
            {"big_lds", &t.big_lds, 0, 65536, 1}, {"vp_big_lds", &t.vp_big_lds, 0, 65536, 1}, {"small_lds", &t.small_lds, 0, 65536, 1},
            {"vp_small_lds", &t.vp_small_lds, 0, 65536, 1}, {"cut_big_lds", &t.cut_big_lds, 0, 65536, 1}, {"vp_cut_big_lds", &t.vp_cut_big_lds, 0, 65536, 1},
            {"cut_small_lds", &t.cut_small_lds, 0, 65536, 1}, {"vp_cut_small_lds", &t.vp_cut_small_lds, 0, 65536, 1}, {"cull_lds", &t.cull_lds, 0, 65000, 1}, {"vp_cull_lds", &t.vp_cull_lds, 0, 65000, 1},
            {"resolve_lds", &t.resolve_lds, 0, 61440, 1}, {"big_grid", &t.big_grid, 256, 65536, 1},
            {"small_grid", &t.small_grid, R3N_SUBQ, 32768, R3N_SUBQ}, {"timed_pipeline", &t.timed_pipeline, 0, 1, 1},
            {"comm_serial", &t.comm_serial, 0, 1, 1}, {"prio_main", &t.prio_main, 0, 2, 1}, {"prio_shade", &t.prio_shade, 0, 2, 1}, {"prio_aux", &t.prio_aux, 0, 2, 1}};
        bool known = false;
        for (auto &k : keys)
            if (key == k.name) {
                if (val < k.lo || val > k.hi || val % k.step) return fail(c, R3N_ERR_INVALID_ARG, "tuning: value out of range for " + key);
                *k.p = (uint32_t)val;
                known = true;
            }
        if (!known) return fail(c, R3N_ERR_INVALID_ARG, "tuning: unknown key " + key);
        at = end == std::string::npos ? text.size() : end;
    }
    c->tune = t;
    return R3N_OK;
}

}

extern "C" int r3n_internal_set_tuning(r3n_ctx *c, const char *kv) { return c ? apply_tuning(c, kv) : R3N_ERR_INVALID_ARG; }
extern "C" int r3n_internal_read_timeline(r3n_ctx *c, float *out, int max) { return c && out ? read_timeline(c, out, max) : -1; }
extern "C" int r3n_internal_live_resources(uint64_t out[4]) {
    if (!out) return R3N_ERR_INVALID_ARG;
    for (int k = 0; k < 4; ++k) out[k] = hip_owned::live_resources[k].load();
    return R3N_OK;
}

__global__ __launch_bounds__(256) static void k_frame_clear(uint32_t *__restrict__ a, size_t a_words, uint32_t *__restrict__ b, size_t b_words,
                                                            uint32_t *__restrict__ c3, size_t c_words) {
    const uint4 z = make_uint4(0u, 0u, 0u, 0u);
    const size_t stride = (size_t)gridDim.x * 256u, t = (size_t)blockIdx.x * 256u + threadIdx.x;
    for (size_t i = t; i < a_words / 4u; i += stride) reinterpret_cast<uint4 *>(a)[i] = z;
    for (size_t i = t; i < b_words / 4u; i += stride) reinterpret_cast<uint4 *>(b)[i] = z;
    for (size_t i = t; i < c_words / 4u; i += stride) reinterpret_cast<uint4 *>(c3)[i] = z;
    if (t < 4u) {
        if ((a_words & ~(size_t)3u) + t < a_words) a[(a_words & ~(size_t)3u) + t] = 0u;
        if ((b_words & ~(size_t)3u) + t < b_words) b[(b_words & ~(size_t)3u) + t] = 0u;
        if ((c_words & ~(size_t)3u) + t < c_words) c3[(c_words & ~(size_t)3u) + t] = 0u;
    }
}

extern "C" {

const char *r3n_create_error(void) { return g_create_error.c_str(); }

r3n_ctx *r3n_create(int hip_device, const r3n_config *config) {
    int n = 0;
    hipError_t e = hipGetDeviceCount(&n);
    if (e != hipSuccess || n == 0) {
        g_create_error = std::string("no HIP device: ") + hipGetErrorString(e);
        return nullptr;
    }
    if (hip_device < 0 || hip_device >= n) { g_create_error = "hip_device out of range"; return nullptr; }
    e = hipSetDevice(hip_device);
    if (e != hipSuccess) { g_create_error = std::string("hipSetDevice: ") + hipGetErrorString(e); return nullptr; }
    hipDeviceProp_t prop;
    e = hipGetDeviceProperties(&prop, hip_device);
    if (e != hipSuccess) { g_create_error = std::string("hipGetDeviceProperties: ") + hipGetErrorString(e); return nullptr; }
    if (std::string(prop.gcnArchName).rfind("gfx950", 0) != 0) {
        g_create_error = std::string("this build targets gfx950 (MI355X) only; device is ") + prop.gcnArchName;
        return nullptr;
    }
    r3n_ctx *c = new r3n_ctx();
    c->device = hip_device;
    if (config && config->struct_size >= sizeof(r3n_config) && config->max_big_items)
        c->big_capacity = std::max(1024u, config->max_big_items / R3N_BIGQ);
    if (config && config->struct_size >= sizeof(r3n_config) && config->shade_mode <= R3N_SHADE_FAST) c->shade_mode = config->shade_mode;
    if (const char *et = std::getenv("R3N_TUNE"))
        if (apply_tuning(c, et) != R3N_OK) {
            g_create_error = "R3N_TUNE: " + c->err;
            delete c;
            return nullptr;
        }
    e = c->stream.create(hipStreamNonBlocking, (int)c->tune.prio_main - 1);
    if (e != hipSuccess) {
        g_create_error = std::string("stream creation: ") + hipGetErrorString(e);
        delete c;
        return nullptr;
    }
    if (c->stage.alloc((size_t)r3n_ctx::kStageSlots * r3n_ctx::kStageSlotBytes, hipHostMallocDefault) != hipSuccess ||
        c->stage_half_done[0].create(hipEventDisableTiming) != hipSuccess ||
        c->stage_half_done[1].create(hipEventDisableTiming) != hipSuccess) {
        g_create_error = "pinned staging ring allocation failed";
        r3n_destroy(c);
        return nullptr;
    }
// ... 1038 lines not shown
    std::vector<uint32_t> block;
    vertex_block::layout layout{};
    if (!texel_compact::lay_out(plan, block, layout)) return fail(c, R3N_ERR_CAPACITY, "mesh compact: more than 2^31 wave slots of copy work in one call");
    const texel_compact::Move &last = plan.moves.back();
    if ((last.src + last.words) * 4u > c->mesh.bytes) return fail(c, R3N_ERR_STATE, "mesh compact: a live block ends outside the mesh buffer");
    std::vector<mesh_reloc::Move> rmoves;
    rmoves.reserve(plan.moves.size());
    for (const texel_compact::Move &m : plan.moves) rmoves.push_back(mesh_reloc::Move{m.src, m.dst, m.words});
    std::vector<mesh_reloc::Entry> table;
    if (!mesh_reloc::build_table(rmoves, table)) return fail(c, R3N_ERR_STATE, "mesh compact: a move outside 32-bit word addresses");
    block.resize((block.size() + 3u) & ~(size_t)3u, 0u);
    const size_t table_at = block.size();
    block.resize(table_at + table.size() * 4u);
    std::memcpy(block.data() + table_at, table.data(), table.size() * sizeof(mesh_reloc::Entry));

    HIP_TRY(c, hipSetDevice(c->device));
    if (!c->tex_stream) HIP_TRY(c, c->tex_stream.create(hipStreamNonBlocking));
    const uint64_t syncs_before = c->sync_serial;
    TRY(sync_all(c));
    mesh_note_syncs(c);
    TRY(grow_texture_scratch(c, c->tex_stage, (size_t)std::max<uint64_t>(plan.scratch_words, 1) * 4u));
    TRY(grow_texture_scratch(c, c->tex_jobs, block.size() * 4u));

    uint32_t *pool = c->mesh.as<uint32_t>(), *scratch = c->tex_stage.as<uint32_t>();
    const uint32_t *jobs = c->tex_jobs.as<uint32_t>();
    hipError_t e = hipMemcpyAsync(c->tex_jobs.p, block.data(), block.size() * 4u, hipMemcpyHostToDevice, c->tex_stream);
    for (size_t i = 0; i < plan.launches.size() && e == hipSuccess; ++i) {
        const texel_compact::Launch &l = plan.launches[i];
        e = (hipError_t)r3n_internal_move_segments(jobs, layout.o_first, layout.o_inst, (uint32_t)l.first_wave, (uint32_t)l.waves,
                                                   l.kind == texel_compact::SCATTER ? scratch : pool, l.kind == texel_compact::GATHER ? scratch : pool,
                                                   c->tex_stream);
    }
    uint64_t launches = plan.launches.size();
    bool relocated = false;
    if (e == hipSuccess && c->capacity && c->objects.p) {
        for (Event &ev : c->mesh_reloc_ev)
            if (!ev && e == hipSuccess) e = ev.create();
        if (e == hipSuccess) e = hipEventRecord(c->mesh_reloc_ev[0], c->tex_stream);
        if (e == hipSuccess) e = (hipError_t)r3n_internal_relocate_objects(c->objects.as<uint32_t>(), c->capacity, jobs + table_at, (uint32_t)table.size(), c->tex_stream);
        if (e == hipSuccess) e = hipEventRecord(c->mesh_reloc_ev[1], c->tex_stream);
        relocated = e == hipSuccess;
        ++launches;
    }
    const hipError_t e2 = hipStreamSynchronize(c->tex_stream);
    if (relocated && e2 == hipSuccess) {
        float ms = 0.0f;
        if (hipEventElapsedTime(&ms, c->mesh_reloc_ev[0], c->mesh_reloc_ev[1]) == hipSuccess) res.relocate_ns = (uint64_t)((double)ms * 1e6);
    }
    if (e != hipSuccess) return fail(c, R3N_ERR_HIP, std::string("mesh compact: ") + hipGetErrorString(e));
    if (e2 != hipSuccess) return fail(c, R3N_ERR_HIP, std::string("mesh compact: ") + hipGetErrorString(e2));
    texel_compact::rebuild(c->mesh_alloc, plan);
    c->mesh_blocks.clear();
    for (const texel_compact::Live &t : plan.live) c->mesh_blocks[t.start] = t.words;
    c->h_skin_inputs.clear();
    ++c->main_epoch;
    for (size_t i = 0; i < plan.moves.size(); ++i)
        moves_out[i] = r3n_mesh_move24{plan.moves[i].src * 4u, plan.moves[i].dst * 4u, plan.moves[i].words};
    res.blocks_moved = plan.moves.size();
    res.words_moved = plan.words_moved;
    res.passes = plan.passes.size();
    res.kernel_launches = launches;
    res.full_syncs = c->sync_serial - syncs_before;
    res.pool_words_after = c->mesh_alloc.end();
    res.free_ranges_after = c->mesh_alloc.free_ranges();
    if (out) *out = res;
    ++c->mesh_stats.compact_calls;
    c->mesh_stats.launches += launches;
    c->mesh_stats.full_waits += res.full_syncs;
    return R3N_OK;
}

int r3n_mesh_stats(r3n_ctx *c, r3n_mesh_counters *out, int reset) {
    if (!c || (!out && !reset)) return fail(c, R3N_ERR_INVALID_ARG, "mesh stats: null");
    if (out) {
        *out = c->mesh_stats;
        out->blocks_live = c->mesh_blocks.size();
        out->live_words = 0;
        for (const auto &kv : c->mesh_blocks) out->live_words += kv.second;
        out->pool_words = c->mesh_alloc.end();
        out->free_ranges = c->mesh_alloc.free_ranges();
        out->buffer_words = c->mesh.bytes / 4u;
    }
    if (reset) c->mesh_stats = r3n_mesh_counters{};
    return R3N_OK;
}

int r3n_lights_write(r3n_ctx *c, const void *dir, uint64_t dir_bytes, const void *point, uint64_t point_bytes) {
    if (!c) return R3N_ERR_INVALID_ARG;
    auto take = [&](std::vector<uint8_t> &h, const char *list, const void *src, uint64_t bytes, uint32_t stride, uint32_t cap) -> int {
        if (!src || bytes < 16) { h.assign(16, 0); return R3N_OK; }
        uint32_t count;
        std::memcpy(&count, src, 4);
        if ((uint64_t)count * stride + 16 > bytes) return fail(c, R3N_ERR_INVALID_ARG, std::string("lights write: ") + list + " light list: count exceeds buffer");
        if (count > cap) return fail(c, R3N_ERR_UNSUPPORTED, std::string("lights write: ") + list + " light list: more lights than the LDS light list holds");
        h.assign(static_cast<const uint8_t *>(src), static_cast<const uint8_t *>(src) + 16u + (size_t)count * stride);
        return R3N_OK;
    };
    std::vector<uint8_t> new_dir, new_point;
    TRY(take(new_dir, "directional", dir, dir_bytes, 128, R3N_MAX_DIR_LIGHTS));
    TRY(take(new_point, "point", point, point_bytes, 32, R3N_MAX_POINT_LIGHTS));
    if (new_dir != c->h_dir || new_point != c->h_point) ++c->lights_version;
    c->h_dir.swap(new_dir);
    c->h_point.swap(new_point);
    return R3N_OK;
}

static int frame_begin_impl(r3n_ctx *c, const r3n_frame_uniforms496 *u, uint32_t w, uint32_t h, uint32_t samples,
                            const float clear_color[4], uint32_t atlas_w, uint32_t atlas_h, const r3n_frame_desc *d) {
    if (!c || !u || !clear_color || !w || !h) return fail(c, R3N_ERR_INVALID_ARG, "frame_begin: bad args");
    if (samples != 1 && samples != 4) return fail(c, R3N_ERR_INVALID_ARG, "frame_begin: samples must be 1 or 4 (SampleCount::One | Four)");
    if (w > 65535 || h > 65535) return fail(c, R3N_ERR_UNSUPPORTED, "frame_begin: target larger than 65535");
    if ((uint64_t)w * h * samples >= (1ull << 29) || (uint64_t)atlas_w * atlas_h >= (1ull << 30) || atlas_w > 65535 || atlas_h > 65535)
        return fail(c, R3N_ERR_UNSUPPORTED, "frame_begin: target of 2^29 samples or more / shadow atlas of 2^30 texels or more");
    HIP_TRY(c, hipSetDevice(c->device));
    c->width = w; c->height = h; c->samples = samples; c->atlas_w = atlas_w; c->atlas_h = atlas_h;
    std::memcpy(c->clear, clear_color, 16);
    const int hs = (int)(c->frame_no % (uint64_t)r3n_ctx::kFbHost);
    c->slot = (int)(c->frame_no++ & 1u);
    std::swap(c->vis, c->alt_vis);
    std::swap(c->atlas, c->alt_atlas);
    if (c->overlap && c->multi_stream) std::swap(c->tri_rec, c->alt_tri_rec);
    std::swap(c->viewport.baked, c->alt_vp_baked);
    uint8_t *dev = c->fb_dev[c->slot].as<uint8_t>();
    c->fu.p = dev + r3n_ctx::kFbUniforms;
    c->dir_buf.p = dev + r3n_ctx::kFbDir;
    c->point_buf.p = dev + r3n_ctx::kFbPoint;
    c->viewport.d_hdr.p = dev + r3n_ctx::kFbViewportHdr; c->viewport.d_hdr.bytes = 256;
    for (auto &kv : c->shadows) { kv.second.d_hdr.p = dev + r3n_ctx::kFbShadowHdr + 256u * (size_t)kv.first; kv.second.d_hdr.bytes = 256; }
    uint32_t *const slot_counts = c->big_count_all.as<uint32_t>() + (size_t)c->slot * r3n_ctx::kBigCountWords;
    for (int lane = 0; lane < 1 + R3N_QLANES; ++lane) c->big_count[lane].p = slot_counts + (size_t)lane * 64 * R3N_BIGQ;
    if (c->shade_pending[c->slot]) {
        HIP_TRY(c, hipStreamWaitEvent(c->stream, c->shade_done[c->slot], 0));
        c->shade_pending[c->slot] = false;
    }
    if (c->fb_pending[hs]) {
        HIP_WAIT(c, hipEventSynchronize(c->fb_ev[hs]));
        c->fb_pending[hs] = false;
    }
    uint8_t *host = c->fb_host[hs].as<uint8_t>();
    std::memcpy(host + r3n_ctx::kFbUniforms, u, sizeof *u);
    if (c->h_dir.size() < 16) c->h_dir.assign(16, 0);
    if (c->h_point.size() < 16) c->h_point.assign(16, 0);
    std::memcpy(host + r3n_ctx::kFbDir, c->h_dir.data(), c->h_dir.size());
    size_t upto = r3n_ctx::kFbShadowHdr;
    if (d) {
        std::memcpy(host + r3n_ctx::kFbViewportHdr, d->viewport_header, sizeof(r3n_camera_header240));
        for (uint32_t v = 0; v < d->n_shadow_views; ++v)
            std::memcpy(host + r3n_ctx::kFbShadowHdr + 256u * (size_t)v, &d->shadow_views[v].header, sizeof(r3n_camera_header240));
        upto += 256u * (size_t)d->n_shadow_views;
    }
    HIP_TRY(c, hipMemcpyAsync(dev, host, upto, hipMemcpyHostToDevice, c->stream));
    if (c->slot_lights_version[c->slot] != c->lights_version) {
        std::memcpy(host + r3n_ctx::kFbPoint, c->h_point.data(), c->h_point.size());
        HIP_TRY(c, hipMemcpyAsync(dev + r3n_ctx::kFbPoint, host + r3n_ctx::kFbPoint, c->h_point.size(), hipMemcpyHostToDevice, c->stream));
        c->slot_lights_version[c->slot] = c->lights_version;
    }
    HIP_TRY(c, hipEventRecord(c->fb_ev[hs], c->stream));
    c->fb_pending[hs] = true;
    const size_t npix = (size_t)w * h;
    TRY(ensure(c, c->vis, npix * samples * 8, false, -1));
    TRY(ensure(c, c->hdr16, npix * 8, false, -1));
    TRY(ensure(c, c->out8, npix * 4, false, -1));
    build_hiz_desc(c->hizd, w, h);
    TRY(ensure(c, c->hiz, hiz_elements(c->hizd) * 4, false, -1));
    const size_t apix = (size_t)std::max(1u, atlas_w) * std::max(1u, atlas_h);
    TRY(ensure(c, c->atlas, apix * 4, false, -1));
// ... 422 lines not shown
    TriCullArgs a{};
    a.hdr = s->d_hdr.as<r3n_camera_header240>();
    a.objects = c->objects.as<r3n_object128>();
    a.mesh = c->mesh.as<uint32_t>();
    a.baked = s->baked.as<r3n_baked128>();
    a.material_keys = c->material_keys.as<uint8_t>();
    a.n_materials = c->n_materials;
    a.vis_list = s->vis_list.as<r3n_vis_entry>();
    a.first_entry = s->first_entry.as<uint32_t>();
    a.counts = s->counts[cur].as<r3n_cull_counts>();
    a.prev_slot_base = (viewport && s->has_prev) ? s->slot_base[prev].as<uint32_t>() : nullptr;
    a.prev_mask = (viewport && s->has_prev) ? s->mask[prev].as<unsigned long long>() : nullptr;
    a.mask = s->mask[cur].as<unsigned long long>();
    a.predicted = s->predicted[cur].as<r3n_tri_ref8>();
    a.residual = viewport ? s->residual.as<r3n_tri_ref8>() : nullptr;
    a.sub_counts = s->sub_counts[cur].as<r3n_sub_counts>();
    a.subcap = subcap;
    a.hiz.data = c->hiz.as<float>();
    a.hiz.d = c->hizd;
    const uint32_t grid = std::max(1u, std::min(chunks, 4096u));
    {
        Timed t(c, R3N_STAGE_TRIANGLE_CULL, stream);
        hipLaunchKernelGGL(k_triangle_cull, dim3(grid), dim3(256), viewport ? c->tune.vp_cull_lds : c->tune.cull_lds, stream, a);
    }
    TRY(check_launch(c, "k_triangle_cull"));
    s->culled = true;
    s->last = cur;
    return R3N_OK;
}

int r3n_hi_z(r3n_ctx *c) {
    if (!c || !c->in_frame) return fail(c, R3N_ERR_STATE, "hi_z: outside a frame");
    HIP_TRY(c, hipSetDevice(c->device));
    Timed t(c, R3N_STAGE_HIZ);
    uint32_t levels = 0;
    while (levels < 4u && levels + 1u < c->hizd.mips && ((c->width >> levels) % 2u == 0u) && ((c->height >> levels) % 2u == 0u) &&
           (c->width >> levels) >= 2u && (c->height >> levels) >= 2u)
        ++levels;
    hipLaunchKernelGGL(k_hiz_head, dim3((c->width + 31u) / 32u, (c->height + 31u) / 32u), dim3(256), 0, c->stream,
                       c->vis.as<unsigned long long>(), c->hiz.as<float>(), c->hizd, levels, c->hiz_plane_ready ? 0u : c->samples);
    c->hiz_plane_ready = false;
    uint32_t first = levels + 1u;
    if (first < c->hizd.mips) {
        const uint32_t dw = std::max(1u, c->width >> first), dh = std::max(1u, c->height >> first);
        if ((size_t)dw * dh > 2304u) {
            const uint32_t sw = std::max(1u, c->width >> (first - 1u)), sh = std::max(1u, c->height >> (first - 1u));
            hipLaunchKernelGGL(k_hiz_downsample, dim3((dw + 15u) / 16u, (dh + 15u) / 16u), dim3(256), 0, c->stream, c->hiz.as<float>() + c->hizd.offset[first - 1u],
                               c->hiz.as<float>() + c->hizd.offset[first], sw, sh, dw, dh);
            ++first;
        }
    }
    if (first < c->hizd.mips) {
        const uint32_t n0 = std::max(1u, c->width >> first) * std::max(1u, c->height >> first);
        hipLaunchKernelGGL(k_hiz_tail, dim3(1), dim3(n0 <= 2304u ? 256 : 1024), 0, c->stream, c->hiz.as<float>(), c->hizd, first);
    }
    return check_launch(c, "hi_z");
}

int r3n_shadow_viewport(r3n_ctx *c, r3n_camera cam, uint32_t x, uint32_t y, uint32_t size) {
    if (!c || cam == R3N_CAMERA_VIEWPORT) return fail(c, R3N_ERR_INVALID_ARG, "shadow_viewport: needs a shadow camera");
    CamState *s = find_cam(c, cam, true);
    if (!s) return fail(c, R3N_ERR_INVALID_ARG, "shadow_viewport: bad camera");
    s->vp_x = x; s->vp_y = y; s->vp_size = size;
    return R3N_OK;
}

static int forward_blend(r3n_ctx *c);

static bool cutout_alpha_short(r3n_ctx *c) {
    if (!c->cutout_short_dirty) return c->cutout_short;
    bool ok = c->n_texels <= (1ull << 30);
    for (uint32_t i = 0; ok && i < c->n_materials && i < c->h_materials.size(); ++i) {
        const r3n_material208 &m = c->h_materials[i];
        if (i >= c->h_material_key.size() || c->h_material_key[i] != R3N_KEY_CUTOUT) continue;
        if (!(m.flags & R3N_FLAGS_ALBEDO_ACTIVE) || m.textures[0] == 0u) continue;
        const uint32_t id = m.textures[0];
        ok = id <= c->n_textures && id <= c->h_tex_short.size() && c->h_tex_short[id - 1u] != 0 && !(m.flags & R3N_FLAGS_NEAREST);
    }
    c->cutout_short = ok;
    c->cutout_short_dirty = false;
    return ok;
}

int r3n_forward(r3n_ctx *c, r3n_camera cam, uint32_t pass, uint32_t source, uint32_t key) {
    if (!c || pass > R3N_PASS_FORWARD || source > R3N_SOURCE_RESIDUAL || key > R3N_KEY_BLEND)
        return fail(c, R3N_ERR_INVALID_ARG, "forward: bad args");
    if (!c->in_frame) return fail(c, R3N_ERR_STATE, "forward: outside a frame");
    if (key == R3N_KEY_BLEND) c->sky_window = false;
    CamState *s = find_cam(c, cam, false);
    if (!s || !s->has_hdr || c->capacity == 0) return R3N_OK;
    key_census(c);
    if ((source == R3N_SOURCE_PREDICTED ? s->key_objects[1 - s->cur][key] : c->key_objects[key]) == 0) return R3N_OK;
    const bool viewport = cam == R3N_CAMERA_VIEWPORT;
    if ((pass == R3N_PASS_FORWARD) != viewport) return fail(c, R3N_ERR_UNSUPPORTED, "forward: FORWARD needs the viewport, DEPTH a shadow camera");
    if (key == R3N_KEY_BLEND) {
        if (!viewport || source != R3N_SOURCE_RESIDUAL) return fail(c, R3N_ERR_INVALID_ARG, "forward: the blend routine draws the viewport's residual source (base.rs:451-465)");
        HIP_TRY(c, hipSetDevice(c->device));
        return forward_blend(c);
    }
    HIP_TRY(c, hipSetDevice(c->device));
    int idx;
    const r3n_tri_ref8 *list;
    const uint32_t *sub_counts;
    if (source == R3N_SOURCE_PREDICTED) {
        if (!s->has_prev) return R3N_OK;
        idx = 1 - s->cur;
        list = s->predicted[idx].as<r3n_tri_ref8>();
        sub_counts = &s->sub_counts[idx].as<r3n_sub_counts>()->n[0][0][0];
    } else {
        if (!s->culled) return R3N_OK;
        idx = s->cur;
        list = viewport ? s->residual.as<r3n_tri_ref8>() : s->predicted[idx].as<r3n_tri_ref8>();
        sub_counts = &s->sub_counts[idx].as<r3n_sub_counts>()->n[viewport ? 1 : 0][0][0];
    }
    RasterArgs a{};
    a.hdr = s->d_hdr.as<r3n_camera_header240>();
    a.objects = c->objects.as<r3n_object128>();
    a.mesh = c->mesh.as<uint32_t>();
    a.baked = s->baked.as<r3n_baked128>();
    a.materials = c->materials.as<r3n_material208>();
    a.material_keys = c->material_keys.as<uint8_t>();
    a.n_materials = c->n_materials;
    a.tri_base = c->tri_base.as<uint32_t>();
    a.list = list;
    a.sub_counts = sub_counts;
    a.subcap = s->subcap[idx];
    a.key = key;
    const int lane = cam_lane(c, cam);
    hipStream_t stream = lane_stream(c, lane);
    a.big_items = c->big_items[lane].as<r3n_big_item>();
    const uint32_t fwd = std::min(c->forward_index_lane[lane]++, 63u);
    a.big_count = c->big_count[lane].as<uint32_t>() + (size_t)fwd * R3N_BIGQ;
    a.big_capacity = c->big_capacity;
    a.big_uv = c->big_uv[lane].as<r3n_big_uv>();
    a.tex = texture_args(c);
    const uint32_t small_grid = c->tune.small_grid;
    TRY(fork_lane(c, lane));
    if (fwd == 63u) HIP_TRY(c, hipMemsetAsync(a.big_count, 0, R3N_BIGQ * 4, stream));
    a.row_begin = 0; a.row_end = 0xFFFFFFFFu;
    if (viewport) {
        a.vp_x = 0; a.vp_y = 0; a.vp_w = c->width; a.vp_h = c->height; a.target_pitch = c->width;
        a.vis = c->vis.as<unsigned long long>();
        if (c->shard_rows) { a.row_begin = std::min(c->row_begin, c->height); a.row_end = std::min(c->row_end, c->height); }
        const bool tex = key == R3N_KEY_CUTOUT && c->n_textures > 0;
        const bool nocut = key != R3N_KEY_CUTOUT;
        auto launch = [&](auto small, auto big) {
            { Timed t(c, nocut ? R3N_STAGE_RASTER : R3N_STAGE_RASTER_CUT, stream); hipLaunchKernelGGL(small, dim3(small_grid), dim3(256), nocut ? c->tune.vp_small_lds : c->tune.vp_cut_small_lds, stream, a); }
            { Timed t(c, nocut ? R3N_STAGE_RASTER_BIG : R3N_STAGE_RASTER_BIG_CUT, stream); hipLaunchKernelGGL(big, dim3(c->tune.big_grid), dim3(256), nocut ? c->tune.vp_big_lds : c->tune.vp_cut_big_lds, stream, a); }
        };
        const bool shorta = tex && cutout_alpha_short(c);
        if (c->samples == 4) {
            if (shorta) launch(k_raster_small<false, 4, true, false, true>, k_raster_big<false, 4, true, false, false, true>);
            else if (tex) launch(k_raster_small<false, 4, true>, k_raster_big<false, 4, true>);
            else if (nocut) launch(k_raster_small<false, 4, false, true>, k_raster_big<false, 4, false, false, true>);
            else launch(k_raster_small<false, 4, false>, k_raster_big<false, 4, false>);
        } else {
            if (shorta) launch(k_raster_small<false, 1, true, false, true>, k_raster_big<false, 1, true, false, false, true>);
            else if (tex) launch(k_raster_small<false, 1, true>, k_raster_big<false, 1, true>);
            else if (nocut) launch(k_raster_small<false, 1, false, true>, k_raster_big<false, 1, false, false, true>);
            else launch(k_raster_small<false, 1, false>, k_raster_big<false, 1, false>);
        }
    } else {
        if (s->vp_size == 0 || s->vp_x + s->vp_size > c->atlas_w || s->vp_y + s->vp_size > c->atlas_h)
            return fail(c, R3N_ERR_STATE, "forward: shadow viewport not set or outside the atlas");
        a.vp_x = s->vp_x; a.vp_y = s->vp_y; a.vp_w = s->vp_size; a.vp_h = s->vp_size; a.target_pitch = c->atlas_w;
        if (c->fused_frame) { a.row_begin = std::min(s->band_begin, s->vp_size); a.row_end = std::min(s->band_end, s->vp_size); }
        a.depth = c->atlas.as<uint32_t>();
        const bool tex = key == R3N_KEY_CUTOUT && c->n_textures > 0;
        if (tex && cutout_alpha_short(c)) {
            { Timed t(c, R3N_STAGE_SHADOW_RASTER, stream); hipLaunchKernelGGL((k_raster_small<true, 1, true, false, true>), dim3(small_grid), dim3(256), c->tune.cut_small_lds, stream, a); }
            { Timed t(c, R3N_STAGE_SHADOW_RASTER_BIG, stream); hipLaunchKernelGGL((k_raster_big<true, 1, true, false, false, true>), dim3(c->tune.big_grid), dim3(256), c->tune.cut_big_lds, stream, a); }
        } else if (tex) {
            { Timed t(c, R3N_STAGE_SHADOW_RASTER, stream); hipLaunchKernelGGL((k_raster_small<true, 1, true>), dim3(small_grid), dim3(256), c->tune.cut_small_lds, stream, a); }
            { Timed t(c, R3N_STAGE_SHADOW_RASTER_BIG, stream); hipLaunchKernelGGL((k_raster_big<true, 1, true>), dim3(c->tune.big_grid), dim3(256), c->tune.cut_big_lds, stream, a); }
        } else if (key != R3N_KEY_CUTOUT) {
            { Timed t(c, R3N_STAGE_SHADOW_RASTER, stream); hipLaunchKernelGGL((k_raster_small<true, 1, false, true>), dim3(small_grid), dim3(256), c->tune.small_lds, stream, a); }
            { Timed t(c, R3N_STAGE_SHADOW_RASTER_BIG, stream); hipLaunchKernelGGL((k_raster_big<true, 1, false, false, true>), dim3(c->tune.big_grid), dim3(256), c->tune.big_lds, stream, a); }
        } else {
            { Timed t(c, R3N_STAGE_SHADOW_RASTER, stream); hipLaunchKernelGGL((k_raster_small<true, 1, false>), dim3(small_grid), dim3(256), c->tune.cut_small_lds, stream, a); }
            { Timed t(c, R3N_STAGE_SHADOW_RASTER_BIG, stream); hipLaunchKernelGGL((k_raster_big<true, 1, false>), dim3(c->tune.big_grid), dim3(256), c->tune.cut_big_lds, stream, a); }
        }
    }
    return check_launch(c, "raster");
}

static int refresh_material_classes(r3n_ctx *c) {
    if (!c->classes_dirty) return R3N_OK;
    const uint32_t n = c->n_materials;
    c->h_materials.resize(n, r3n_material208{});
    std::vector<uint32_t> feat(std::max(n, 1u), R3N_FEAT_ALL);
    const bool small_pool = c->n_texels <= (1ull << 30);
    uint32_t variants = 0;
    for (uint32_t i = 0; i < n; ++i) {
        const r3n_material208 &m = c->h_materials[i];
        uint32_t f = r3n_material_features(m);
        for (int k = 0; k < 10; ++k) {
            const uint32_t id = m.textures[k];
            if (id && (!small_pool || id > c->n_textures || id > c->h_tex_short.size() || !c->h_tex_short[id - 1u])) f |= R3N_FEAT_TEX_GENERAL;
        }
        feat[i] = f;
        variants |= 1u << r3n_variant_of(f);
    }
    TRY(ensure(c, c->material_feat, feat.size() * 4, false, -1));
    HIP_TRY(c, hipMemcpyAsync(c->material_feat.p, feat.data(), feat.size() * 4, hipMemcpyHostToDevice, c->stream));
    HIP_WAIT(c, hipStreamSynchronize(c->stream));
    c->resolve_variants = variants;
    c->classes_dirty = false;
    return R3N_OK;
}

static ShadeArgs make_shade_args(r3n_ctx *c, uint32_t r0, uint32_t r1) {
    CamState &s = c->viewport;
    ShadeArgs a{};
    a.vis = c->vis.as<unsigned long long>();
    a.width = c->width; a.height = c->height; a.row_begin = r0; a.row_end = r1;
    a.fu = c->fu.as<r3n_frame_uniforms496>();
    a.hdr = s.d_hdr.as<r3n_camera_header240>();
    a.objects = c->objects.as<r3n_object128>();
    a.mesh = c->mesh.as<uint32_t>();
    a.baked = s.baked.as<r3n_baked128>();
    a.materials = c->materials.as<r3n_material208>();
    a.n_materials = c->n_materials;
    a.tri_base = c->tri_base.as<uint32_t>();
    a.slot_table = c->slot_table.as<uint32_t>();
    a.slot_table_size = c->slot_table_size;
    a.dir_buf = c->dir_buf.as<uint8_t>();
    a.point_buf = c->point_buf.as<uint8_t>();
    a.atlas = c->atlas.as<float>();
    a.atlas_w = std::max(1u, c->atlas_w); a.atlas_h = std::max(1u, c->atlas_h);
    std::memcpy(a.clear, c->clear, 16);
    a.hdr_out = c->hdr16.as<ushort4>();
    a.ldr_out = c->out8.as<uchar4>();
    a.srgb_lut = c->srgb_lut.as<unsigned char>();
    a.out_bgr = (c->output_format & 1u) != 0u;
    a.tex = texture_args(c);
    a.samples_out = nullptr;
    a.tri_rec = nullptr;
    a.seen = nullptr;
    a.resolve_lds = c->tune.resolve_lds;
    a.total_tris = (uint32_t)c->total_tris;
    a.view_lights = nullptr;
    a.material_feat = nullptr;
    a.variants = 0u;
    return a;
}

int r3n_resolve_opaque(r3n_ctx *c) {
    if (!c || !c->in_frame) return fail(c, R3N_ERR_STATE, "resolve_opaque: outside a frame");
    HIP_TRY(c, hipSetDevice(c->device));
    const uint32_t r0 = std::min(c->row_begin, c->height), r1 = std::min(c->row_end, c->height);
    c->sky_window = r1 <= r0;
    c->resolve_on_shade = false;
    if (r1 <= r0) return R3N_OK;
    CamState &s = c->viewport;
    if (!s.has_hdr && c->capacity) return fail(c, R3N_ERR_STATE, "resolve_opaque: viewport uniforms not baked");
    const bool use_records = c->total_tris > 0 && (uint64_t)c->total_tris * sizeof(TriRecord) <= (8ull << 30);
    const uint64_t npix_all = (uint64_t)c->width * c->height;
    const bool blend_samples = c->samples == 4 && c->blend_tris > 0;
    const bool split = c->samples == 4 && use_records && !blend_samples && npix_all < (1ull << 29);
// ... 600 lines not shown
        TRY(r3n_exchange_depth(c, &plane, &n));
        Timed t(c, R3N_STAGE_EXCHANGE_DEPTH, c->stream);
        TRY(comm_order_begin(c, c->stream));
        NCCL_TRY(c, rccl().AllReduce(plane, plane, (size_t)n, ncclFloat32, ncclMax, c->comm.main, c->stream));
        return comm_order_end(c, c->stream);
    }
    Timed t(c, R3N_STAGE_EXCHANGE_DEPTH, c->stream);
    TRY(comm_order_begin(c, c->stream));
    NCCL_TRY(c, rccl().AllReduce(c->vis.p, c->vis.p, (size_t)c->width * c->height * c->samples, ncclUint64, ncclMax, c->comm.main, c->stream));
    return comm_order_end(c, c->stream);
}
static int comm_reduce_pass2(r3n_ctx *c) {
    const uint32_t world = c->comm.world, rank = c->comm.rank, h = c->height;
    const size_t row_keys = (size_t)c->width * c->samples;
    unsigned long long *keys = c->vis.as<unsigned long long>();
    Timed t(c, R3N_STAGE_EXCHANGE_KEYS, c->stream);
    TRY(comm_order_begin(c, c->stream));
    if (h % world == 0) {
        const size_t chunk = (size_t)(h / world) * row_keys;
        NCCL_TRY(c, rccl().ReduceScatter(keys, keys + (size_t)rank * chunk, chunk, ncclUint64, ncclMax, c->comm.main, c->stream));
    } else {
        NCCL_TRY(c, rccl().AllReduce(keys, keys, (size_t)h * row_keys, ncclUint64, ncclMax, c->comm.main, c->stream));
    }
    return comm_order_end(c, c->stream);
}
static int comm_gather_rows(r3n_ctx *c) {
    void *out = nullptr, *sp = nullptr;
    uint64_t bytes = 0;
    TRY(r3n_output_buffer_async(c, &out, &bytes, &sp));
    {
        Timed t(c, R3N_STAGE_EXCHANGE_ROWS, (hipStream_t)sp);
        TRY(comm_gather_bands(c, out, (size_t)c->width * 4, c->comm.rows, (hipStream_t)sp));
    }
    return r3n_output_work_enqueued(c);
}

int r3n_render_frame(r3n_ctx *c, const r3n_frame_desc *d) {
    if (!c || !d || d->struct_size < sizeof(r3n_frame_desc)) return fail(c, R3N_ERR_INVALID_ARG, "render_frame: bad descriptor");
    if (!d->uniforms || !d->viewport_header || (d->n_shadow_views && !d->shadow_views) || d->n_shadow_views > R3N_MAX_SHADOW_VIEWS)
        return fail(c, R3N_ERR_INVALID_ARG, "render_frame: null uniforms / headers, or too many shadow views");
    if (c->in_frame) return fail(c, R3N_ERR_STATE, "render_frame: a frame is already open");
    const bool native = c->comm.on;
    crumb(c, "render_frame", d->width, d->height);
    if (native) {
        if (d->exchange) return fail(c, R3N_ERR_INVALID_ARG, "render_frame: an exchange callback AND r3n_comm_init communicators");
        band_rows(d->height, c->comm.world, c->comm.rank, c->row_begin, c->row_end);
    }
    for (uint32_t v = 0; v < d->n_shadow_views; ++v)
        if (d->shadow_views[v].header.shadow_index != v) return fail(c, R3N_ERR_INVALID_ARG, "render_frame: shadow view i must carry shadow_index i");
    if (d->directional_buffer) TRY(r3n_lights_write(c, d->directional_buffer, d->directional_bytes, d->point_buffer, d->point_bytes));
    TRY(frame_begin_impl(c, d->uniforms, d->width, d->height, d->samples, d->clear_color, d->shadow_atlas_width, d->shadow_atlas_height, d));
    c->viewport.hdr_frame = c->frame_no;
    for (uint32_t v = 0; v < d->n_shadow_views; ++v)
        if (CamState *s = find_cam(c, v, true)) {
            s->hdr_frame = c->frame_no;
            s->d_hdr.p = c->fb_dev[c->slot].as<uint8_t>() + r3n_ctx::kFbShadowHdr + 256u * (size_t)v;
            s->d_hdr.bytes = 256;
        }
    struct Closer {
        r3n_ctx *c; bool armed = true;
        ~Closer() { if (armed && c->in_frame) { const std::string keep = c->err; (void)close_frame(c); c->err = keep; } }
    } closer{c};
    struct Fused { r3n_ctx *c; ~Fused() { c->fused_frame = false; } } fused{c};
    c->fused_frame = true;
    if (d->exchange) c->exchanged_this_frame = true;
    const bool masked = native || (d->flags & R3N_FRAME_SHADOW_MASK) != 0u;
    auto mine = [&](uint32_t v) {
        if (native) return shadow_part_of(c->comm.world, d->n_shadow_views, c->comm.rank, v) >= 0;
        return !masked || ((d->shadow_view_mask >> v) & 1ull) != 0ull;
    };
    for (uint32_t v = 0; v < d->n_shadow_views; ++v) {
        const r3n_shadow_view272 &sv = d->shadow_views[v];
        TRY(r3n_shadow_viewport(c, v, sv.x, sv.y, sv.size));
        {
            CamState *s = find_cam(c, v, true);
            if (!s) return fail(c, R3N_ERR_INVALID_ARG, "render_frame: bad shadow camera");
            s->band_begin = 0; s->band_end = 0xFFFFFFFFu;
            const int part = native ? shadow_part_of(c->comm.world, d->n_shadow_views, c->comm.rank, v) : -1;
            if (part >= 0) band_rows(sv.size, shadow_parts(c->comm.world, d->n_shadow_views), (uint32_t)part, s->band_begin, s->band_end);
        }
        if (masked) TRY(r3n_set_camera_object_range(c, v, mine(v) ? 0u : 0xFFFFFFFFu, mine(v) ? 0xFFFFFFFEu : 0xFFFFFFFFu));
    }
    if (d->n_skeletons) TRY(r3n_skinning(c, d->skin_inputs, d->n_skeletons, d->joint_matrices, d->n_joint_matrices));
    auto shadow_nodes = [&]() -> int {
        for (uint32_t v = 0; v < d->n_shadow_views; ++v)
            if (mine(v)) TRY(r3n_uniform_bake(c, v, &d->shadow_views[v].header));
        for (uint32_t v = 0; v < d->n_shadow_views; ++v)
            if (mine(v)) TRY(r3n_cull(c, v));
        for (uint32_t v = 0; v < d->n_shadow_views; ++v)
            if (mine(v)) {
                TRY(r3n_forward(c, v, R3N_PASS_DEPTH, R3N_SOURCE_RESIDUAL, R3N_KEY_OPAQUE));
                TRY(r3n_forward(c, v, R3N_PASS_DEPTH, R3N_SOURCE_RESIDUAL, R3N_KEY_CUTOUT));
            }
        if (d->exchange && d->n_shadow_views && d->exchange(d->exchange_user, R3N_EXCHANGE_SHADOW) != 0)
            return fail(c, R3N_ERR_STATE, "render_frame: the shadow exchange callback failed");
        return R3N_OK;
    };
    auto viewport_pass1 = [&]() -> int {
        TRY(r3n_uniform_bake(c, R3N_CAMERA_VIEWPORT, d->viewport_header));
        TRY(r3n_forward(c, R3N_CAMERA_VIEWPORT, R3N_PASS_FORWARD, R3N_SOURCE_PREDICTED, R3N_KEY_OPAQUE));
        TRY(r3n_forward(c, R3N_CAMERA_VIEWPORT, R3N_PASS_FORWARD, R3N_SOURCE_PREDICTED, R3N_KEY_CUTOUT));
        return R3N_OK;
    };
    if (d->flags & R3N_FRAME_VIEWPORT_FIRST) { TRY(viewport_pass1()); TRY(shadow_nodes()); }
    else { TRY(shadow_nodes()); TRY(viewport_pass1()); }
    if (d->exchange && d->exchange(d->exchange_user, R3N_EXCHANGE_PASS1) != 0) return fail(c, R3N_ERR_STATE, "render_frame: the pass-1 exchange callback failed");
    if (native) TRY(c->comm.by_objects ? comm_reduce_pass1(c) : comm_exchange_pass1(c));
    if (native && d->n_shadow_views) TRY(comm_exchange_shadows(c, d));
    TRY(r3n_hi_z(c));
    TRY(r3n_cull(c, R3N_CAMERA_VIEWPORT));
    TRY(r3n_forward(c, R3N_CAMERA_VIEWPORT, R3N_PASS_FORWARD, R3N_SOURCE_RESIDUAL, R3N_KEY_OPAQUE));
    TRY(r3n_forward(c, R3N_CAMERA_VIEWPORT, R3N_PASS_FORWARD, R3N_SOURCE_RESIDUAL, R3N_KEY_CUTOUT));
    if (d->exchange && d->exchange(d->exchange_user, R3N_EXCHANGE_PASS2) != 0) return fail(c, R3N_ERR_STATE, "render_frame: the pass-2 exchange callback failed");
    if (native && c->comm.by_objects) TRY(comm_reduce_pass2(c));
    TRY(r3n_resolve_opaque(c));
    TRY(r3n_skybox(c));
    TRY(r3n_forward(c, R3N_CAMERA_VIEWPORT, R3N_PASS_FORWARD, R3N_SOURCE_RESIDUAL, R3N_KEY_BLEND));
    TRY(r3n_tonemap(c, nullptr, 0));
    if (native) TRY(comm_gather_rows(c));
    closer.armed = false;
    crumb(c, "render_frame enqueued");
    return r3n_frame_end(c);
}

int r3n_set_object_range(r3n_ctx *c, uint32_t begin, uint32_t end) {
    if (!c || begin > end) return fail(c, R3N_ERR_INVALID_ARG, "set_object_range: begin > end");
    c->range_begin = begin; c->range_end = end;
    return R3N_OK;
}
int r3n_set_object_owners(r3n_ctx *c, const uint8_t *owners, uint32_t n, uint32_t rank) {
    if (!c) return R3N_ERR_INVALID_ARG;
    HIP_TRY(c, hipSetDevice(c->device));
    TRY(sync_all(c));
    if (!owners || n == 0) {
        (void)c->owners.reset();
        c->owners_n = 0;
        return R3N_OK;
    }
    if (n < c->capacity) return fail(c, R3N_ERR_INVALID_ARG, "set_object_owners: one owner byte per object slot (n >= capacity)");
    TRY(ensure(c, c->owners, n, false, -1));
    HIP_TRY(c, hipMemcpy(c->owners.p, owners, n, hipMemcpyHostToDevice));
    c->owners_n = n;
    c->owner_rank = rank;
    return R3N_OK;
}
int r3n_set_camera_object_range(r3n_ctx *c, r3n_camera cam, uint32_t begin, uint32_t end) {
    if (!c) return R3N_ERR_INVALID_ARG;
    CamState *s = find_cam(c, cam, true);
    if (!s) return fail(c, R3N_ERR_INVALID_ARG, "set_camera_object_range: bad camera");
    if (begin == 0xFFFFFFFFu && end == 0xFFFFFFFFu) { s->range_set = false; return R3N_OK; }
    if (begin > end) return fail(c, R3N_ERR_INVALID_ARG, "set_camera_object_range: begin > end");
    s->range_set = true; s->range_begin = begin; s->range_end = end;
    return R3N_OK;
}
int r3n_exchange_depth(r3n_ctx *c, void **depth_f32, uint64_t *count) {
    if (!c || !c->in_frame || !c->vis.p) return fail(c, R3N_ERR_STATE, "exchange_depth: outside a frame");
    if (c->samples != 1) return fail(c, R3N_ERR_UNSUPPORTED, "exchange_depth: single-sample targets only (a multisampled pass-1 exchange carries the keys)");
    HIP_TRY(c, hipSetDevice(c->device));
    const size_t n = (size_t)c->width * c->height;
    {
        Timed t(c, R3N_STAGE_HIZ);
        hipLaunchKernelGGL(k_hiz_mip0, dim3((unsigned)std::min<size_t>((n + 255) / 256, 65535u * 16u)), dim3(256), 0, c->stream,
                           c->vis.as<unsigned long long>(), c->hiz.as<float>(), n);
    }
    TRY(check_launch(c, "k_hiz_mip0"));
    c->hiz_plane_ready = true;
    c->exchanged_this_frame = true;
    if (depth_f32) *depth_f32 = c->hiz.p;
    if (count) *count = n;
    return R3N_OK;
}
int r3n_exchange_buffers(r3n_ctx *c, void **vis, uint64_t *vis_count, void **atlas, uint64_t *atlas_count) {
    if (!c || !c->vis.p) return fail(c, R3N_ERR_STATE, "exchange_buffers: no frame targets yet");
    TRY(join_lanes(c));
    c->exchanged_this_frame = true;
// ... 426 lines not shown
```

rend3_amd/renderer.py:

```python
import ctypes

import os

import numpy as np

from . import _ffi, host

f32 = np.float32
INVALID = 0xFFFFFFFF
OPAQUE, CUTOUT, BLEND = 0, 1, 2

FLAGS_ALBEDO_ACTIVE = 0x0001
FLAGS_ALBEDO_BLEND = 0x0002
FLAGS_ALBEDO_VERTEX_SRGB = 0x0004
FLAGS_AOMR_COMBINED = 0x0040
FLAGS_AOMR_SPLIT = 0x0100
FLAGS_CC_GLTF_COMBINED = 0x0400
FLAGS_BICOMPONENT_NORMAL = 0x0008
FLAGS_SWIZZLED_NORMAL = 0x0010
FLAGS_YDOWN_NORMAL = 0x0020
FLAGS_AOMR_SWIZZLED_SPLIT = 0x0080
FLAGS_AOMR_BW_SPLIT = 0x0200
FLAGS_CC_GLTF_SPLIT = 0x0800
FLAGS_CC_BW_SPLIT = 0x1000
# ... 646 lines not shown
    def _remove_mesh_block(self, what, block):
        if self._mesh_upload != "stream":
            raise ValueError(f"{what} needs Renderer(mesh_upload='stream'): the append path gives no words back")
        offs = np.array([block], dtype=np.uint64)
        self._check(self.lib.r3n_mesh_blocks_remove(self.ctx, _ffi.ptr(offs), 1), "r3n_mesh_blocks_remove")
        self._mesh_edits = True

    def _enabled_objects(self):
        return [meta for meta in self.object_meta.values() if meta.get("enabled")]

    def remove_mesh(self, h):
        if self._mesh_upload != "stream":
            raise ValueError("remove_mesh needs Renderer(mesh_upload='stream'): the append path gives no words back")
        if self.meshes[h] is None:
            raise ValueError("remove_mesh: the mesh was removed already")
        if (any(meta.get("mesh") == h for meta in self._enabled_objects()) or any(sk is not None and sk["mesh"] == h for sk in self.skeletons)
                or any(inst is not None and inst["mesh"] == h for inst in self.morphs)):
            raise ValueError("remove_mesh: an enabled object, a skeleton or a morph instance still names the mesh")
        self._remove_mesh_block("remove_mesh", self.meshes[h].block)
        self.meshes[h] = None

    def remove_skeleton(self, h):
        if self._mesh_upload != "stream":
            raise ValueError("remove_skeleton needs Renderer(mesh_upload='stream'): the append path gives no words back")
        if self.skeletons[h] is None:
            raise ValueError("remove_skeleton: the skeleton was removed already")
        if any(meta.get("skeleton") == h for meta in self._enabled_objects()):
            raise ValueError("remove_skeleton: an enabled object is still bound to the skeleton")
        self._remove_mesh_block("remove_skeleton", self.skeletons[h]["block"])
        self.skeletons[h] = None
        self._pose_state.pop(h, None)
        self._skin_inputs = None
        self.world_version += 1

    def remove_morph_instance(self, h):
        if self._mesh_upload != "stream":
            raise ValueError("remove_morph_instance needs Renderer(mesh_upload='stream'): the append path gives no words back")
        if self.morphs[h] is None:
            raise ValueError("remove_morph_instance: the instance was removed already")
        if (any(h in (meta.get("morph"), meta.get("morph_instance")) for meta in self._enabled_objects())
                or any(sk is not None and sk["morph"] == h for sk in self.skeletons)):
            raise ValueError("remove_morph_instance: an enabled object or a skeleton is still bound to the instance")
        self._remove_mesh_block("remove_morph_instance", self.morphs[h]["block"])
        self.morphs[h] = None
        self._morph_dirty.discard(h)
        self.world_version += 1

    def compact_meshes(self, max_words=0, stage_words=0):
        if self._mesh_upload != "stream":
            raise ValueError("compact_meshes needs Renderer(mesh_upload='stream'): the append path lays its buffer out densely")
        capacity = max(self.mesh_stats()["blocks_live"], 1)
        moves = (_ffi.MeshMove24 * capacity)()
        opts = _ffi.MeshCompactOpts(max_words=int(max_words), stage_words=int(stage_words))
        out = _ffi.MeshCompactResult()
        self._check(self.lib.r3n_mesh_compact(self.ctx, ctypes.byref(opts), ctypes.byref(out), moves, capacity), "r3n_mesh_compact")
        res = {name: int(getattr(out, name)) for name, _ in _ffi.MeshCompactResult._fields_}
        res["moves"] = np.array([(mv.old_byte_offset, mv.new_byte_offset, mv.padded_words) for mv in moves[:res["blocks_moved"]]],
                                dtype=np.uint64).reshape(-1, 3)
        if res["blocks_moved"]:
            self._apply_mesh_moves(res["moves"])
        return res

    def _apply_mesh_moves(self, moves):
        def one(off):
            return int(relocate_offsets(np.uint32(off), moves))
        for m in self.meshes:
            if m is not None:
                _shift_mesh(m, one)
                m.block = one(m.block)
        for entry in list(self.skeletons) + list(self.morphs):
            if entry is not None:
                entry["out_off"] = [int(o) for o in relocate_offsets(entry["out_off"], moves)]
                entry["block"] = one(entry["block"])
        if getattr(self, "_skin_inputs", None) is not None:
            self._skin_inputs[:, :8] = relocate_offsets(self._skin_inputs[:, :8], moves)
        for rec in self.dirty_objects.values():
            rec[20] = relocate_offsets(rec[20], moves, words=True)
            rec[23:29] = relocate_offsets(rec[23:29], moves)

    def mesh_stats(self, reset=False):
        out = _ffi.MeshCounters()
        self._check(self.lib.r3n_mesh_stats(self.ctx, ctypes.byref(out), 1 if reset else 0), "r3n_mesh_stats")
        return {name: int(getattr(out, name)) for name, _ in _ffi.MeshCounters._fields_}

    def readback_objects(self, first_slot=0, n=None):
        n = self.capacity - first_slot if n is None else int(n)
        out = np.zeros((max(n, 1), 32), dtype=np.uint32)
        if n:
            self._check(self.lib.r3n_readback_objects(self.ctx, int(first_slot), _ffi.ptr(out), n), "r3n_readback_objects")
        return out[:n]

    @property
    def texture_upload(self):
        return self._texture_upload

    @texture_upload.setter
    def texture_upload(self, mode):
        if mode not in ("whole", "stream"):
            raise ValueError("texture_upload: 'whole' or 'stream'")
        if mode != self._texture_upload and (len(self.tex_descs) or self._tex_live):
            raise ValueError("texture_upload cannot change once textures exist")
        self._texture_upload = mode

    @property
    def texture_compact(self):
        return self._texture_compact

    @texture_compact.setter
    def texture_compact(self, fraction):
        if fraction is not None and not (0.0 < float(fraction) <= 1.0):
            raise ValueError("texture_compact: None or a fraction in (0, 1]")
        self._texture_compact = None if fraction is None else float(fraction)

    def add_texture_2d(self, rgba8, srgb=True, mip_count=1, mip_source="uploaded"):
        data, w, h, mips, stored = host.prepare_texture(rgba8, srgb, mip_count, mip_source)
        return self._append_texture(data, w, h, mips, 1 if srgb else 0, stored)

    def add_texture_2d_encoded(self, fmt, width, height, levels, generate_mips=False):
        from . import containers
        if generate_mips:
            if not containers.generate_mips_allowed(fmt) or len(levels) != 1:
                raise ValueError("mips are generated for single-level 8-bit uncompressed textures only")
            mips = int(max(width, height)).bit_length()
            return self._append_texture(np.frombuffer(levels[0], dtype=np.uint8), width, height, mips, fmt, 1 if mips > 1 else 0)
        for k, lv in enumerate(levels):
            if len(lv) != containers.level_bytes(fmt, max(1, width >> k), max(1, height >> k)):
                raise ValueError(f"level {k}: wrong byte count for its extent")
        return self._append_texture(np.frombuffer(b"".join(levels), dtype=np.uint8), width, height, len(levels), fmt)

    def _append_texture(self, data_u8, w, h, mips, fmt, stored=0):
        if self._texture_upload == "stream":
            if self._tex_tails:
                self._flush_textures()
            slot = self._take_texture_slot(mips)
            self._tex_queue.append((slot, (w, h, mips, fmt, stored), np.array(data_u8, dtype=np.uint8)))
            return slot
        start = (self.tex_used + 3) & ~3
        end = start + len(data_u8)
        if end > len(self.tex_pool):
            grown = np.zeros(max(2 * len(self.tex_pool), end), dtype=np.uint8)
            grown[: self.tex_used] = self.tex_pool[: self.tex_used]
            self.tex_pool = grown
        self.tex_pool[start:end] = data_u8
        self.tex_used = end
        desc = np.array([[start, w, h, mips, fmt, stored, 0, 0]], dtype=np.uint32)
        self.tex_descs = np.ascontiguousarray(np.concatenate([self.tex_descs, desc]))
        self._tex_dirty = True
        return len(self.tex_descs) - 1

    def _take_texture_slot(self, mips):
        slot = self._tex_live.index(False) if False in self._tex_live else len(self._tex_live)
        if slot == len(self._tex_live):
            self._tex_live.append(True)
            self._tex_mips.append(0)
        self._tex_live[slot] = True
        self._tex_mips[slot] = int(mips)
        return slot

    def add_texture_2d_from_texture(self, src, start_mip, mip_count=None):
        if self._texture_upload != "stream":
            raise ValueError("add_texture_2d_from_texture needs Renderer(texture_upload='stream'): the whole-array path keeps no resident pool to copy from")
        src, start_mip = int(src), int(start_mip)
        if not (0 <= src < len(self._tex_live)) or not self._tex_live[src]:
            raise ValueError(f"add_texture_2d_from_texture: handle {src} holds no texture")
        mips = self._tex_mips[src]
        count = mips - start_mip if mip_count is None else int(mip_count)
# ... 872 lines not shown
```

Baseline: 10270 Mpixels/s.

## Defer shadow triangles predicted occluded by previous frame's shadow depth pyramid

Adds temporal occlusion culling to the opaque shadow depth pass. When a shadow view's projection differs from the previous frame's only by a whole-pixel translation, small planar triangles whose nearest depth lies behind the shifted min-depth pyramid are placed in a deferred list instead of being rasterised. After the main pass, a min-depth pyramid is built from the current shadow atlas and the deferred triangles are retested against it, then rasterised only if they survive. This is meant to cut rasteriser work for occluded shadow casters, at the cost of an extra pyramid build, a deferred pass and a late big-triangle launch per view.

Measured after the change: 11130 Mpixels/s, median of 6. 8.3% higher.

```diff
diff --git a/bindings/rend3-amd-sys/src/lib.rs b/bindings/rend3-amd-sys/src/lib.rs
--- a/bindings/rend3-amd-sys/src/lib.rs
+++ b/bindings/rend3-amd-sys/src/lib.rs
@@ -480,6 +480,17 @@
 
 #[repr(C)]
 #[derive(Clone, Copy)]
+pub struct r3n_shadow_occlusion_counters {
+    pub active: u32,
+    pub predicted: u32,
+    pub deferred: u32,
+    pub dropped: u32,
+    pub survivors: u32,
+    pub capacity: u32,
+}
+
+#[repr(C)]
+#[derive(Clone, Copy)]
 pub struct r3n_tri_ref {
     pub object: u32,
     pub triangle: u32,
@@ -575,6 +586,7 @@
     pub fn r3n_hdr_write(ctx: *mut r3n_ctx, rgba16f: *const u16, first_pixel: u64, n_pixels: u64) -> c_int;
     pub fn r3n_frame_end(ctx: *mut r3n_ctx) -> c_int;
     pub fn r3n_render_frame(ctx: *mut r3n_ctx, desc: *const r3n_frame_desc) -> c_int;
+    pub fn r3n_shadow_occlusion_stats(ctx: *mut r3n_ctx, camera: u32, out: *mut r3n_shadow_occlusion_counters) -> c_int;
     pub fn r3n_set_object_range(ctx: *mut r3n_ctx, begin: u32, end: u32) -> c_int;
     pub fn r3n_set_object_owners(ctx: *mut r3n_ctx, owners: *const u8, n: u32, rank: u32) -> c_int;
     pub fn r3n_set_shard_mode(ctx: *mut r3n_ctx, mode: u32) -> c_int;
diff --git a/include/r3n.h b/include/r3n.h
--- a/include/r3n.h
+++ b/include/r3n.h
@@ -361,6 +361,10 @@
     void *exchange_user;
 } r3n_frame_desc;
 int r3n_render_frame(r3n_ctx *ctx, const r3n_frame_desc *desc);
+typedef struct r3n_shadow_occlusion_counters {
+    uint32_t active, predicted, deferred, dropped, survivors, capacity;
+} r3n_shadow_occlusion_counters;
+int r3n_shadow_occlusion_stats(r3n_ctx *ctx, r3n_camera camera, r3n_shadow_occlusion_counters *out);
 
 int r3n_set_object_range(r3n_ctx *ctx, uint32_t begin, uint32_t end);
 int r3n_set_object_owners(r3n_ctx *ctx, const uint8_t *owners, uint32_t n, uint32_t rank);
diff --git a/rend3_amd/_ffi.py b/rend3_amd/_ffi.py
--- a/rend3_amd/_ffi.py
+++ b/rend3_amd/_ffi.py
@@ -72,6 +72,7 @@
     "r3n_hdr_write": (cint, [vp, vp, u64, u64]),
     "r3n_frame_end": (cint, [vp]),
     "r3n_render_frame": (cint, [vp, vp]),
+    "r3n_shadow_occlusion_stats": (cint, [vp, u32, vp]),
     "r3n_set_object_range": (cint, [vp, u32, u32]),
     "r3n_set_object_owners": (cint, [vp, vp, u32, u32]),
     "r3n_exchange_buffers": (cint, [vp, vp, vp, vp, vp]),
@@ -201,6 +202,10 @@
                                          "blocks_live", "live_words", "pool_words", "free_ranges", "buffer_words")]
 
 
+class ShadowOcclusionCounters(ctypes.Structure):
+    _fields_ = [(name, u32) for name in ("active", "predicted", "deferred", "dropped", "survivors", "capacity")]
+
+
 class TextureTail16(ctypes.Structure):
     _fields_ = [("dst_slot", u32), ("src_slot", u32), ("start_mip", u32), ("mip_count", u32)]
 
diff --git a/rend3_amd/csrc/device_math.h b/rend3_amd/csrc/device_math.h
--- a/rend3_amd/csrc/device_math.h
+++ b/rend3_amd/csrc/device_math.h
@@ -124,6 +124,7 @@
     float z[3];
     float det;
     bool valid;
+    bool planar;
 };
 
 R3N_DEV void setup_triangle(const float p[3][4], float half_w, float half_h, bool positive_visible, TriSetup &ts) {
@@ -170,6 +171,7 @@
             planar = true;
         }
     }
+    ts.planar = planar;
     if (!planar) {
         ts.z[0] = ((ts.e[0][0] * zc[0] + ts.e[1][0] * zc[1]) + ts.e[2][0] * zc[2]) / det;
         ts.z[1] = ((ts.e[0][1] * zc[0] + ts.e[1][1] * zc[1]) + ts.e[2][1] * zc[2]) / det;
diff --git a/rend3_amd/csrc/kernels_raster.h b/rend3_amd/csrc/kernels_raster.h
--- a/rend3_amd/csrc/kernels_raster.h
+++ b/rend3_amd/csrc/kernels_raster.h
@@ -1,6 +1,30 @@
 #pragma once
 #include "device_math.h"
 #include "texture.h"
+
+struct r3n_deferred32 {
+    uint32_t object, triangle, xy0, xy1;
+    float bound;
+    uint32_t _pad[3];
+};
+#define R3N_OCC_SUBLISTS 32
+#define R3N_OCC_CTL_STRIDE 64
+#define R3N_OCC_CTL_COUNT(parity, q) (((parity) * R3N_OCC_SUBLISTS + (q)) * R3N_OCC_CTL_STRIDE)
+#define R3N_OCC_CTL_LAST (2 * R3N_OCC_SUBLISTS * R3N_OCC_CTL_STRIDE)
+#define R3N_OCC_CTL_DROPPED (R3N_OCC_CTL_LAST + R3N_OCC_SUBLISTS)
+#define R3N_OCC_CTL_SURVIVORS (R3N_OCC_CTL_DROPPED + 1)
+#define R3N_OCC_CTL_WORDS (R3N_OCC_CTL_LAST + 2 * R3N_OCC_SUBLISTS)
+struct OcclusionArgs {
+    float *pyramid;
+    uint32_t *ctl;
+    r3n_deferred32 *list;
+    uint32_t capacity;
+    uint32_t log2_size;
+    uint32_t parity;
+    uint32_t predict;
+    int shift_x, shift_y;
+    float shift_z;
+};
 
 struct RasterArgs {
     const r3n_camera_header240 *hdr;
@@ -31,6 +55,7 @@
     uint32_t *frag_head;
     uint32_t *status;
     uint32_t row_begin, row_end;
+    OcclusionArgs occ;
 };
 
 R3N_DEV float cutout_alpha(uint32_t mat_flags, float mat_alpha, float tex_alpha, float vertex_alpha) {
@@ -66,10 +91,33 @@
     bool cutout;
     float thr[3];
     int x0, y0, x1, y1;
+    float bound;
 };
-
-
-template <bool DEPTH_ONLY, bool TEX, bool NOCUT = false>
+#define R3N_OCC_NEVER 2.0f
+#define R3N_OCC_MAX_BOX 64
+
+R3N_DEV float occ_depth_bound(const TriSetup &ts, int x0, int y0, int x1, int y1) {
+    const float px = (float)(f32_positive(ts.z[0]) ? x1 : x0) + 0.5f, py = (float)(f32_positive(ts.z[1]) ? y1 : y0) + 0.5f;
+    return fminf(frag_depth(ts, px, py), 1.0f);
+}
+R3N_DEV uint32_t occ_level_offset(uint32_t ls, uint32_t L) {
+    uint32_t off = 0u;
+    for (uint32_t l = 2u; l < L; ++l) off += 1u << (2u * (ls - l));
+    return off;
+}
+R3N_DEV float occ_tile_min(const OcclusionArgs &o, int x0, int y0, int x1, int y1) {
+    const uint32_t m = (uint32_t)max(x1 - x0, y1 - y0);
+    const uint32_t L = max(2u, 32u - (uint32_t)__clz((int)m));
+    const float *lv = o.pyramid + occ_level_offset(o.log2_size, L);
+    const uint32_t n = o.log2_size - L;
+    const uint32_t tx0 = (uint32_t)x0 >> L, tx1 = (uint32_t)x1 >> L, r0 = ((uint32_t)y0 >> L) << n, r1 = ((uint32_t)y1 >> L) << n;
+    const float a = lv[r0 + tx0], b = lv[r0 + tx1], c = lv[r1 + tx0], d = lv[r1 + tx1];
+    return fminf(fminf(a, b), fminf(c, d));
+}
+
+
+
+template <bool DEPTH_ONLY, bool TEX, bool NOCUT = false, bool OCC = false>
 R3N_DEV bool prepare_triangle(const RasterArgs &a, uint32_t obj, uint32_t tri, bool positive_visible, TriWork &tw) {
     const r3n_object128 &ob = a.objects[obj];
     const uint4 of = *reinterpret_cast<const uint4 *>(reinterpret_cast<const char *>(&ob) + offsetof(r3n_object128, first_index));
@@ -94,6 +142,11 @@
     tw.y0 = max(tw.y0, (int)a.row_begin);
     tw.y1 = min(tw.y1, (int)min(a.row_end, a.vp_h) - 1);
     if (tw.y0 > tw.y1) return false;
+    if (OCC) {
+        const bool can = tw.ts.planar && p[0][3] == 1.0f && p[1][3] == 1.0f && p[2][3] == 1.0f && tw.x1 - tw.x0 < R3N_OCC_MAX_BOX &&
+                         tw.y1 - tw.y0 < R3N_OCC_MAX_BOX;
+        tw.bound = can ? occ_depth_bound(tw.ts, tw.x0, tw.y0, tw.x1, tw.y1) : R3N_OCC_NEVER;
+    }
 #pragma unroll
     for (int i = 0; i < 3; ++i) tw.thr[i] = edge_threshold(tw.ts.e[i][0], tw.ts.e[i][1]);
     tw.cutout = !NOCUT && a.key == R3N_KEY_CUTOUT;
@@ -346,7 +399,51 @@
 #define R3N_FINE_LW_DEPTH 3
 #define R3N_FINE_LW_VIS 3
 
-template <bool DEPTH_ONLY, int S = 1, bool TEX = false, bool NOCUT = false, bool SHORTA = false>
+template <bool DEPTH_ONLY, int S, bool TEX, bool SHORTA>
+R3N_DEV void raster_prepared(const RasterArgs &a, const TriWork &tw, uint32_t bq) {
+    const int bw = tw.x1 - tw.x0 + 1, bh = tw.y1 - tw.y0 + 1;
+    if (bw <= R3N_SMALL_MAX && bh <= R3N_SMALL_MAX) {
+        for (int y = tw.y0; y <= tw.y1; ++y)
+            for (int x = tw.x0; x <= tw.x1; ++x) shade_pixel<DEPTH_ONLY, R3N_PREREAD_SMALL != 0, S, TEX, false, false, SHORTA>(a, tw, x, y);
+    } else {
+        const int ax0 = tw.x0 & ~(R3N_ITEM_ALIGN - 1);
+        const uint32_t tx = (uint32_t)(tw.x1 - ax0 + R3N_TILE) / R3N_TILE, ty = (uint32_t)(bh + (R3N_TILE - 1)) / R3N_TILE;
+        const uint32_t cnt = tx * ty;
+        const uint32_t start = global_add_u32(&a.big_count[bq], cnt);
+        r3n_big_item *big = a.big_items + (size_t)bq * a.big_capacity;
+        for (uint32_t t = 0; t < cnt; ++t) {
+            const uint32_t ix = t % tx, iy = t / tx;
+            const int rx0 = max(ax0 + (int)ix * R3N_TILE, tw.x0), ry0 = tw.y0 + (int)iy * R3N_TILE;
+            const int rx1 = min(ax0 + (int)ix * R3N_TILE + (R3N_TILE - 1), tw.x1), ry1 = min(ry0 + (R3N_TILE - 1), tw.y1);
+            if (start + t < a.big_capacity) {
+                r3n_big_item it;
+#pragma unroll
+                for (int i = 0; i < 3; ++i) {
+#pragma unroll
+                    for (int c = 0; c < 3; ++c) it.e[i][c] = tw.ts.e[i][c];
+                    it.z[i] = tw.ts.z[i];
+                }
+                it.slot1 = DEPTH_ONLY ? 0u : tw.slot1;
+                it.material = tw.material | pack_thresholds(tw.thr);
+                it.xy0 = (uint32_t)rx0 | ((uint32_t)ry0 << 16);
+                it.xy1 = (uint32_t)rx1 | ((uint32_t)ry1 << 16);
+                big[start + t] = it;
+                if (tw.cutout) {
+                    r3n_big_uv bu;
+#pragma unroll
+                    for (int k = 0; k < 3; ++k) { bu.uv[k][0] = tw.uv[k][0]; bu.uv[k][1] = tw.uv[k][1]; bu.va[k] = tw.va[k]; }
+                    bu._pad[0] = bu._pad[1] = bu._pad[2] = 0u;
+                    a.big_uv[(size_t)bq * a.big_capacity + start + t] = bu;
+                }
+            } else {
+                for (int y = ry0; y <= ry1; ++y)
+                    for (int x = rx0; x <= rx1; ++x) shade_pixel<DEPTH_ONLY, R3N_PREREAD_SMALL != 0, S, TEX, false, false, SHORTA>(a, tw, x, y);
+            }
+        }
+    }
+}
+
+template <bool DEPTH_ONLY, int S = 1, bool TEX = false, bool NOCUT = false, bool SHORTA = false, bool OCC = false>
 R3N_DEV void raster_small_body(const RasterArgs &a) {
     const uint32_t q = blockIdx.x % R3N_SUBQ;
     const uint32_t n = a.sub_counts[a.key * R3N_SUBQ + q];
@@ -357,53 +454,106 @@
     for (uint32_t i = (blockIdx.x / R3N_SUBQ) * blockDim.x + threadIdx.x; i < n; i += stride) {
         const r3n_tri_ref8 ref = list[i];
         TriWork tw;
-        if (!prepare_triangle<DEPTH_ONLY, TEX, NOCUT>(a, ref.object, ref.triangle, positive_visible, tw)) continue;
-        const int bw = tw.x1 - tw.x0 + 1, bh = tw.y1 - tw.y0 + 1;
-        if (bw <= R3N_SMALL_MAX && bh <= R3N_SMALL_MAX) {
-            for (int y = tw.y0; y <= tw.y1; ++y)
-                for (int x = tw.x0; x <= tw.x1; ++x) shade_pixel<DEPTH_ONLY, R3N_PREREAD_SMALL != 0, S, TEX, false, false, SHORTA>(a, tw, x, y);
-        } else {
-            const int ax0 = tw.x0 & ~(R3N_ITEM_ALIGN - 1);
-            const uint32_t tx = (uint32_t)(tw.x1 - ax0 + R3N_TILE) / R3N_TILE, ty = (uint32_t)(bh + (R3N_TILE - 1)) / R3N_TILE;
-            const uint32_t cnt = tx * ty;
-            const uint32_t start = global_add_u32(&a.big_count[bq], cnt);
-            r3n_big_item *big = a.big_items + (size_t)bq * a.big_capacity;
-            for (uint32_t t = 0; t < cnt; ++t) {
-                const uint32_t ix = t % tx, iy = t / tx;
-                const int rx0 = max(ax0 + (int)ix * R3N_TILE, tw.x0), ry0 = tw.y0 + (int)iy * R3N_TILE;
-                const int rx1 = min(ax0 + (int)ix * R3N_TILE + (R3N_TILE - 1), tw.x1), ry1 = min(ry0 + (R3N_TILE - 1), tw.y1);
-                if (start + t < a.big_capacity) {
-                    r3n_big_item it;
-#pragma unroll
-                    for (int i = 0; i < 3; ++i) {
-#pragma unroll
-                        for (int c = 0; c < 3; ++c) it.e[i][c] = tw.ts.e[i][c];
-                        it.z[i] = tw.ts.z[i];
-                    }
-                    it.slot1 = DEPTH_ONLY ? 0u : tw.slot1;
-                    it.material = tw.material | pack_thresholds(tw.thr);
-                    it.xy0 = (uint32_t)rx0 | ((uint32_t)ry0 << 16);
-                    it.xy1 = (uint32_t)rx1 | ((uint32_t)ry1 << 16);
-                    big[start + t] = it;
-                    if (tw.cutout) {
-                        r3n_big_uv bu;
-#pragma unroll
-                        for (int k = 0; k < 3; ++k) { bu.uv[k][0] = tw.uv[k][0]; bu.uv[k][1] = tw.uv[k][1]; bu.va[k] = tw.va[k]; }
-                        bu._pad[0] = bu._pad[1] = bu._pad[2] = 0u;
-                        a.big_uv[(size_t)bq * a.big_capacity + start + t] = bu;
-                    }
-                } else {
-                    for (int y = ry0; y <= ry1; ++y)
-                        for (int x = rx0; x <= rx1; ++x) shade_pixel<DEPTH_ONLY, R3N_PREREAD_SMALL != 0, S, TEX, false, false, SHORTA>(a, tw, x, y);
+        if (!prepare_triangle<DEPTH_ONLY, TEX, NOCUT, OCC>(a, ref.object, ref.triangle, positive_visible, tw)) continue;
+        if (OCC && a.occ.predict != 0u && tw.bound <= 1.0f) {
+            const int sx0 = tw.x0 - a.occ.shift_x, sy0 = tw.y0 - a.occ.shift_y, sx1 = tw.x1 - a.occ.shift_x, sy1 = tw.y1 - a.occ.shift_y;
+            const int lim = 1 << a.occ.log2_size;
+            if (sx0 >= 0 && sy0 >= 0 && sx1 < lim && sy1 < lim && tw.bound - a.occ.shift_z < occ_tile_min(a.occ, sx0, sy0, sx1, sy1)) {
+                const uint32_t sub = bq % R3N_OCC_SUBLISTS;
+                const uint32_t at = global_add_u32(&a.occ.ctl[R3N_OCC_CTL_COUNT(a.occ.parity, sub)], 1u);
+                if (at < a.occ.capacity) {
+                    uint4 *rec = reinterpret_cast<uint4 *>(a.occ.list + (size_t)sub * a.occ.capacity + at);
+                    rec[0] = make_uint4(ref.object, ref.triangle,(uint32_t)tw.x0 | ((uint32_t)tw.y0 << 16), (uint32_t)tw.x1 | ((uint32_t)tw.y1 << 16));
+                    rec[1] = make_uint4(__float_as_uint(tw.bound), 0u, 0u, 0u);
+                    continue;
                 }
             }
         }
-    }
-}
-
-template <bool DEPTH_ONLY, int S = 1, bool TEX = false, bool NOCUT = false, bool SHORTA = false>
+        raster_prepared<DEPTH_ONLY, S, TEX, SHORTA>(a, tw, bq);
+    }
+}
+
+template <bool DEPTH_ONLY, int S = 1, bool TEX = false, bool NOCUT = false, bool SHORTA = false, bool OCC = false>
 __global__ __launch_bounds__(256, R3N_SMALL_OCC) void k_raster_small(RasterArgs a) {
-    raster_small_body<DEPTH_ONLY, S, TEX, NOCUT, SHORTA>(a);
+    raster_small_body<DEPTH_ONLY, S, TEX, NOCUT, SHORTA, OCC>(a);
+}
+
+__global__ __launch_bounds__(256) void k_shadow_tile_min(const uint32_t *__restrict__ atlas, uint32_t pitch, uint32_t vp_x, uint32_t vp_y, OcclusionArgs o) {
+    __shared__ float s2[256], s3[64], s4[16], s5[4];
+    const uint32_t ls = o.log2_size, t = threadIdx.x;
+    const uint32_t bx = blockIdx.x & ((1u << (ls - 6u)) - 1u), by = blockIdx.x >> (ls - 6u);
+    {
+        const uint32_t tx = t & 15u, ty = t >> 4;
+        const uint32_t *row = atlas + (size_t)(vp_y + by * 64u + ty * 4u) * pitch + (vp_x + bx * 64u + tx * 4u);
+        float m = INFINITY;
+#pragma unroll
+        for (uint32_t r = 0; r < 4u; ++r) {
+            const float4 v = *reinterpret_cast<const float4 *>(row + (size_t)r * pitch);
+            m = fminf(m, fminf(fminf(v.x, v.y), fminf(v.z, v.w)));
+        }
+        s2[t] = m;
+        o.pyramid[occ_level_offset(ls, 2u) + ((by * 16u + ty) << (ls - 2u)) + bx * 16u + tx] = m;
+    }
+    __syncthreads();
+    if (t < 64u) {
+        const uint32_t cx = t & 7u, cy = t >> 3, at = cy * 32u + cx * 2u;
+        const float m = fminf(fminf(s2[at], s2[at + 1u]), fminf(s2[at + 16u], s2[at + 17u]));
+        s3[t] = m;
+        o.pyramid[occ_level_offset(ls, 3u) + ((by * 8u + cy) << (ls - 3u)) + bx * 8u + cx] = m;
+    }
+    __syncthreads();
+    if (t < 16u) {
+        const uint32_t cx = t & 3u, cy = t >> 2, at = cy * 16u + cx * 2u;
+        const float m = fminf(fminf(s3[at], s3[at + 1u]), fminf(s3[at + 8u], s3[at + 9u]));
+        s4[t] = m;
+        o.pyramid[occ_level_offset(ls, 4u) + ((by * 4u + cy) << (ls - 4u)) + bx * 4u + cx] = m;
+    }
+    __syncthreads();
+    if (t < 4u) {
+        const uint32_t cx = t & 1u, cy = t >> 1, at = cy * 8u + cx * 2u;
+        const float m = fminf(fminf(s4[at], s4[at + 1u]), fminf(s4[at + 4u], s4[at + 5u]));
+        s5[t] = m;
+        o.pyramid[occ_level_offset(ls, 5u) + ((by * 2u + cy) << (ls - 5u)) + bx * 2u + cx] = m;
+    }
+    __syncthreads();
+    if (t == 0u) {
+        o.pyramid[occ_level_offset(ls, 6u) + (by << (ls - 6u)) + bx] = fminf(fminf(s5[0], s5[1]), fminf(s5[2], s5[3]));
+    }
+    if (blockIdx.x == 0u && t < R3N_OCC_SUBLISTS) {
+        o.ctl[R3N_OCC_CTL_LAST + t] = min(o.ctl[R3N_OCC_CTL_COUNT(o.parity, t)], o.capacity);
+        o.ctl[R3N_OCC_CTL_COUNT(o.parity ^ 1u, t)] = 0u;
+        if (t < 2u) o.ctl[R3N_OCC_CTL_DROPPED + t] = 0u;
+    }
+}
+
+__global__ __launch_bounds__(256) void k_shadow_deferred(RasterArgs a) {
+    __shared__ uint32_t tally[2];
+    if (threadIdx.x < 2u) tally[threadIdx.x] = 0u;
+    __syncthreads();
+    const uint32_t q = blockIdx.x % R3N_OCC_SUBLISTS;
+    const uint32_t n = a.occ.ctl[R3N_OCC_CTL_LAST + q];
+    const r3n_deferred32 *list = a.occ.list + (size_t)q * a.occ.capacity;
+    const uint32_t stride = (gridDim.x / R3N_OCC_SUBLISTS) * blockDim.x;
+    const uint32_t bq = __builtin_amdgcn_readfirstlane((blockIdx.x * (blockDim.x >> 6) + (threadIdx.x >> 6)) % R3N_BIGQ);
+    const bool positive_visible = (a.hdr->flags & R3N_PCU_POSITIVE_AREA_VISIBLE) != 0u;
+    uint32_t dropped = 0u, survivors = 0u;
+    for (uint32_t i = (blockIdx.x / R3N_OCC_SUBLISTS) * blockDim.x + threadIdx.x; i < n; i += stride) {
+        const uint4 *rec = reinterpret_cast<const uint4 *>(list + i);
+        const uint4 r = rec[0];
+        const float bound = __uint_as_float(rec[1].x);
+        if (bound < occ_tile_min(a.occ, (int)(r.z & 0xFFFFu), (int)(r.z >> 16), (int)(r.w & 0xFFFFu), (int)(r.w >> 16))) {
+            ++dropped;
+            continue;
+        }
+        ++survivors;
+        TriWork tw;
+        if (!prepare_triangle<true, false, true>(a, r.x, r.y, positive_visible, tw)) continue;
+        raster_prepared<true, 1, false, false>(a, tw, bq);
+    }
+    if (dropped) atomicAdd(&tally[0], dropped);
+    if (survivors) atomicAdd(&tally[1], survivors);
+    __syncthreads();
+    if (threadIdx.x < 2u && tally[threadIdx.x]) (void)global_add_u32(&a.occ.ctl[R3N_OCC_CTL_DROPPED + threadIdx.x], tally[threadIdx.x]);
 }
 struct BlendSetupArgs {
     const uint32_t *order;
diff --git a/rend3_amd/csrc/r3n.hip b/rend3_amd/csrc/r3n.hip
--- a/rend3_amd/csrc/r3n.hip
+++ b/rend3_amd/csrc/r3n.hip
@@ -62,6 +62,12 @@
     bool range_set = false;
     uint32_t range_begin = 0, range_end = 0xFFFFFFFFu;
     uint32_t band_begin = 0, band_end = 0xFFFFFFFFu;
+    DeviceBuffer occ_pyramid, occ_ctl, occ_list;
+    uint32_t occ_capacity = 0, occ_parity = 0;
+    uint64_t occ_frame = ~0ull;
+    uint32_t occ_size = 0;
+    float occ_view_proj[16] = {};
+    uint32_t occ_predicted = 0;
 };
 
 std::string g_create_error;
@@ -75,6 +81,8 @@
 #define R3N_BIG_LDS 40960
 #define R3N_SMALL_LDS 24576
 #define R3N_VIEWPORT_BIG_LDS 49152
+#define R3N_OCC_DEFERRED_GRID 1024
+#define R3N_OCC_LATE_BIG_GRID 256
 #define R3N_QLANES R3N_AUX_STREAMS
 static_assert(R3N_AUX_STREAMS >= 1, "the shadow views draw on auxiliary streams");
 
@@ -94,6 +102,8 @@
     bool always_fork = false;
     bool resolve_classes = true;
     bool fused_frame = false;
+    bool occ_wanted = false, occ_open = false;
+    RasterArgs occ_args{};
     DeviceBuffer alt_vis, alt_atlas, alt_vp_baked;
     static constexpr size_t kFbUniforms = 0, kFbViewportHdr = 512, kFbDir = 768, kFbShadowHdr = 3072,
                             kFbPoint = kFbShadowHdr + 256 * R3N_MAX_SHADOW_VIEWS, kFbBytes = kFbPoint + 8448;
@@ -136,6 +146,7 @@
         uint32_t resolve_lds = 0;
         uint32_t big_grid = R3N_BIG_GRID, small_grid = R3N_SMALL_GRID;
         uint32_t comm_serial = 1;
+        uint32_t shadow_occlusion = 1;
     } tune;
     bool cutout_short_dirty = true, cutout_short = false;
     bool key_census_dirty = true;
@@ -668,7 +679,7 @@
             {"cut_small_lds", &t.cut_small_lds, 0, 65536, 1}, {"vp_cut_small_lds", &t.vp_cut_small_lds, 0, 65536, 1}, {"cull_lds", &t.cull_lds, 0, 65000, 1}, {"vp_cull_lds", &t.vp_cull_lds, 0, 65000, 1},
             {"resolve_lds", &t.resolve_lds, 0, 61440, 1}, {"big_grid", &t.big_grid, 256, 65536, 1},
             {"small_grid", &t.small_grid, R3N_SUBQ, 32768, R3N_SUBQ}, {"timed_pipeline", &t.timed_pipeline, 0, 1, 1},
-            {"comm_serial", &t.comm_serial, 0, 1, 1}, {"prio_main", &t.prio_main, 0, 2, 1}, {"prio_shade", &t.prio_shade, 0, 2, 1}, {"prio_aux", &t.prio_aux, 0, 2, 1}};
+            {"comm_serial", &t.comm_serial, 0, 1, 1}, {"shadow_occlusion", &t.shadow_occlusion, 0, 1, 1}, {"prio_main", &t.prio_main, 0, 2, 1}, {"prio_shade", &t.prio_shade, 0, 2, 1}, {"prio_aux", &t.prio_aux, 0, 2, 1}};
         bool known = false;
         for (auto &k : keys)
             if (key == k.name) {
@@ -1873,6 +1884,26 @@
         out->buffer_words = c->mesh.bytes / 4u;
     }
     if (reset) c->mesh_stats = r3n_mesh_counters{};
+    return R3N_OK;
+}
+
+int r3n_shadow_occlusion_stats(r3n_ctx *c, r3n_camera cam, r3n_shadow_occlusion_counters *out) {
+    if (!c || !out) return fail(c, R3N_ERR_INVALID_ARG, "shadow occlusion stats: null");
+    *out = r3n_shadow_occlusion_counters{};
+    CamState *s = cam == R3N_CAMERA_VIEWPORT ? nullptr : find_cam(c, cam, false);
+    if (!s) return fail(c, R3N_ERR_INVALID_ARG, "shadow occlusion stats: not a shadow camera of this context");
+    if (c->in_frame) return fail(c, R3N_ERR_STATE, "shadow occlusion stats: a frame is open");
+    if (!s->occ_ctl.p || s->occ_frame != c->frame_no) return R3N_OK;
+    std::vector<uint32_t> w(R3N_OCC_CTL_WORDS);
+    HIP_TRY(c, hipSetDevice(c->device));
+    TRY(sync_all(c));
+    HIP_TRY(c, hipMemcpy(w.data(), s->occ_ctl.p, w.size() * 4u, hipMemcpyDeviceToHost));
+    out->active = 1;
+    out->predicted = s->occ_predicted;
+    for (uint32_t q = 0; q < R3N_OCC_SUBLISTS; ++q) out->deferred += w[R3N_OCC_CTL_LAST + q];
+    out->dropped = w[R3N_OCC_CTL_DROPPED];
+    out->survivors = w[R3N_OCC_CTL_SURVIVORS];
+    out->capacity = s->occ_capacity * R3N_OCC_SUBLISTS;
     return R3N_OK;
 }
 
@@ -2461,6 +2492,82 @@
     return ok;
 }
 
+namespace {
+
+static bool occ_view_qualifies(const r3n_ctx *c, const CamState &s) {
+    const uint32_t n = s.vp_size;
+    return n >= 64u && (n & (n - 1u)) == 0u && n <= 32768u && (s.vp_x & 3u) == 0u && (c->atlas_w & 3u) == 0u && s.band_begin == 0u && s.band_end == 0xFFFFFFFFu;
+}
+
+static int shadow_occlusion_begin(r3n_ctx *c, CamState &s, RasterArgs &a) {
+    const uint32_t n = s.vp_size;
+    uint32_t ls = 0;
+    while ((1u << ls) < n) ++ls;
+    size_t floats = 0;
+    for (uint32_t l = 2; l <= 6; ++l) floats += (size_t)1 << (2u * (ls - l));
+    const uint32_t capacity = (uint32_t)std::min<uint64_t>((uint64_t)R3N_SUBQ * a.subcap, (1u << 20) / R3N_OCC_SUBLISTS);
+    TRY(ensure(c, s.occ_pyramid, floats * 4u, false, -1));
+    TRY(ensure(c, s.occ_ctl, R3N_OCC_CTL_WORDS * 4u, false, 0));
+    if (capacity > s.occ_capacity || !s.occ_list.p) {
+        TRY(ensure(c, s.occ_list, (size_t)capacity * R3N_OCC_SUBLISTS * sizeof(r3n_deferred32), false, -1));
+        s.occ_capacity = (uint32_t)(s.occ_list.bytes / sizeof(r3n_deferred32) / R3N_OCC_SUBLISTS);
+    }
+    OcclusionArgs &o = a.occ;
+    o.pyramid = s.occ_pyramid.as<float>();
+    o.ctl = s.occ_ctl.as<uint32_t>();
+    o.list = s.occ_list.as<r3n_deferred32>();
+    o.capacity = s.occ_capacity;
+    o.log2_size = ls;
+    o.parity = s.occ_parity;
+    o.predict = 0u;
+    const float *m = s.hdr.view_proj, *pm = s.occ_view_proj;
+    bool same = s.occ_frame + 1u == c->frame_no && s.occ_size == n;
+    float scale = 0.0f;
+    for (int col = 0; col < 3; ++col)
+        for (int row = 0; row < 3; ++row) scale = std::max(scale, std::fabs(pm[col * 4 + row]));
+    for (int col = 0; col < 3 && same; ++col)
+        for (int row = 0; row < 3; ++row) same = same && std::fabs(m[col * 4 + row] - pm[col * 4 + row]) <= 1e-6f * scale;
+    for (const float *q : {m, pm}) same = same && q[3] == 0.0f && q[7] == 0.0f && q[11] == 0.0f && q[15] == 1.0f;
+    if (same) {
+        const float half = (float)n / 2.0f;
+        const float fx = (m[12] - pm[12]) * half, fy = -(m[13] - pm[13]) * half, fz = m[14] - pm[14];
+        const float rx = std::nearbyint(fx), ry = std::nearbyint(fy);
+        if (std::fabs(fx - rx) <= 1e-3f && std::fabs(fy - ry) <= 1e-3f && std::fabs(rx) < (float)n && std::fabs(ry) < (float)n && fz - fz == 0.0f) {
+            o.predict = 1u;
+            o.shift_x = (int)rx; o.shift_y = (int)ry; o.shift_z = fz;
+        }
+    }
+    s.occ_predicted = o.predict;
+    return R3N_OK;
+}
+
+static int shadow_occlusion_finish(r3n_ctx *c, r3n_camera cam) {
+    if (!c->occ_open) return R3N_OK;
+    c->occ_open = false;
+    CamState *s = find_cam(c, cam, false);
+    if (!s) return R3N_OK;
+    RasterArgs a = c->occ_args;
+    const int lane = cam_lane(c, cam);
+    hipStream_t stream = lane_stream(c, lane);
+    const uint32_t fwd = std::min(c->forward_index_lane[lane]++, 63u);
+    a.big_count = c->big_count[lane].as<uint32_t>() + (size_t)fwd * R3N_BIGQ;
+    if (fwd == 63u) HIP_TRY(c, hipMemsetAsync(a.big_count, 0, R3N_BIGQ * 4, stream));
+    const uint32_t tiles = 1u << (a.occ.log2_size - 6u);
+    {
+        Timed t(c, R3N_STAGE_SHADOW_RASTER, stream);
+        hipLaunchKernelGGL(k_shadow_tile_min, dim3(tiles * tiles), dim3(256), 0, stream, (const uint32_t *)a.depth, a.target_pitch, a.vp_x, a.vp_y, a.occ);
+    }
+    { Timed t(c, R3N_STAGE_SHADOW_RASTER, stream); hipLaunchKernelGGL(k_shadow_deferred, dim3(R3N_OCC_DEFERRED_GRID), dim3(256), 0, stream, a); }
+    { Timed t(c, R3N_STAGE_SHADOW_RASTER_BIG, stream); hipLaunchKernelGGL((k_raster_big<true, 1, false, false, true>), dim3(R3N_OCC_LATE_BIG_GRID), dim3(256), 0, stream, a); }
+    s->occ_parity ^= 1u;
+    s->occ_frame = c->frame_no;
+    s->occ_size = s->vp_size;
+    std::memcpy(s->occ_view_proj, s->hdr.view_proj, sizeof s->occ_view_proj);
+    return check_launch(c, "shadow occlusion");
+}
+
+}
+
 int r3n_forward(r3n_ctx *c, r3n_camera cam, uint32_t pass, uint32_t source, uint32_t key) {
     if (!c || pass > R3N_PASS_FORWARD || source > R3N_SOURCE_RESIDUAL || key > R3N_KEY_BLEND)
         return fail(c, R3N_ERR_INVALID_ARG, "forward: bad args");
@@ -2514,6 +2621,8 @@
     a.big_uv = c->big_uv[lane].as<r3n_big_uv>();
     a.tex = texture_args(c);
     const uint32_t small_grid = c->tune.small_grid;
+    const bool occ = !viewport && c->occ_wanted && key == R3N_KEY_OPAQUE && source == R3N_SOURCE_RESIDUAL;
+    if (occ) TRY(shadow_occlusion_begin(c, *s, a));
     TRY(fork_lane(c, lane));
     if (fwd == 63u) HIP_TRY(c, hipMemsetAsync(a.big_count, 0, R3N_BIGQ * 4, stream));
     a.row_begin = 0; a.row_end = 0xFFFFFFFFu;
@@ -2553,7 +2662,13 @@
             { Timed t(c, R3N_STAGE_SHADOW_RASTER, stream); hipLaunchKernelGGL((k_raster_small<true, 1, true>), dim3(small_grid), dim3(256), c->tune.cut_small_lds, stream, a); }
             { Timed t(c, R3N_STAGE_SHADOW_RASTER_BIG, stream); hipLaunchKernelGGL((k_raster_big<true, 1, true>), dim3(c->tune.big_grid), dim3(256), c->tune.cut_big_lds, stream, a); }
         } else if (key != R3N_KEY_CUTOUT) {
-            { Timed t(c, R3N_STAGE_SHADOW_RASTER, stream); hipLaunchKernelGGL((k_raster_small<true, 1, false, true>), dim3(small_grid), dim3(256), c->tune.small_lds, stream, a); }
+            if (occ) {
+                { Timed t(c, R3N_STAGE_SHADOW_RASTER, stream); hipLaunchKernelGGL((k_raster_small<true, 1, false, true, false, true>), dim3(small_grid), dim3(256), c->tune.small_lds, stream, a); }
+                c->occ_args = a;
+                c->occ_open = true;
+            } else {
+                { Timed t(c, R3N_STAGE_SHADOW_RASTER, stream); hipLaunchKernelGGL((k_raster_small<true, 1, false, true>), dim3(small_grid), dim3(256), c->tune.small_lds, stream, a); }
+            }
             { Timed t(c, R3N_STAGE_SHADOW_RASTER_BIG, stream); hipLaunchKernelGGL((k_raster_big<true, 1, false, false, true>), dim3(c->tune.big_grid), dim3(256), c->tune.big_lds, stream, a); }
         } else {
             { Timed t(c, R3N_STAGE_SHADOW_RASTER, stream); hipLaunchKernelGGL((k_raster_small<true, 1, false>), dim3(small_grid), dim3(256), c->tune.cut_small_lds, stream, a); }
@@ -3320,6 +3435,8 @@
         if (masked) TRY(r3n_set_camera_object_range(c, v, mine(v) ? 0u : 0xFFFFFFFFu, mine(v) ? 0xFFFFFFFEu : 0xFFFFFFFFu));
     }
     if (d->n_skeletons) TRY(r3n_skinning(c, d->skin_inputs, d->n_skeletons, d->joint_matrices, d->n_joint_matrices));
+    const bool occlusion = c->tune.shadow_occlusion != 0u && !native && !d->exchange && !c->shard_rows && c->row_begin == 0u && c->row_end == 0xFFFFFFFFu;
+    c->occ_open = false;
     auto shadow_nodes = [&]() -> int {
         for (uint32_t v = 0; v < d->n_shadow_views; ++v)
             if (mine(v)) TRY(r3n_uniform_bake(c, v, &d->shadow_views[v].header));
@@ -3327,8 +3444,13 @@
             if (mine(v)) TRY(r3n_cull(c, v));
         for (uint32_t v = 0; v < d->n_shadow_views; ++v)
             if (mine(v)) {
-                TRY(r3n_forward(c, v, R3N_PASS_DEPTH, R3N_SOURCE_RESIDUAL, R3N_KEY_OPAQUE));
+                const CamState *s = find_cam(c, v, false);
+                c->occ_wanted = occlusion && s && occ_view_qualifies(c, *s);
+                const int r = r3n_forward(c, v, R3N_PASS_DEPTH, R3N_SOURCE_RESIDUAL, R3N_KEY_OPAQUE);
+                c->occ_wanted = false;
+                TRY(r);
                 TRY(r3n_forward(c, v, R3N_PASS_DEPTH, R3N_SOURCE_RESIDUAL, R3N_KEY_CUTOUT));
+                TRY(shadow_occlusion_finish(c, v));
             }
         if (d->exchange && d->n_shadow_views && d->exchange(d->exchange_user, R3N_EXCHANGE_SHADOW) != 0)
             return fail(c, R3N_ERR_STATE, "render_frame: the shadow exchange callback failed");
diff --git a/rend3_amd/renderer.py b/rend3_amd/renderer.py
--- a/rend3_amd/renderer.py
+++ b/rend3_amd/renderer.py
@@ -752,6 +752,11 @@
         out = _ffi.MeshCounters()
         self._check(self.lib.r3n_mesh_stats(self.ctx, ctypes.byref(out), 1 if reset else 0), "r3n_mesh_stats")
         return {name: int(getattr(out, name)) for name, _ in _ffi.MeshCounters._fields_}
+
+    def shadow_occlusion_stats(self, view):
+        out = _ffi.ShadowOcclusionCounters()
+        self._check(self.lib.r3n_shadow_occlusion_stats(self.ctx, int(view), ctypes.byref(out)), "r3n_shadow_occlusion_stats")
+        return {name: int(getattr(out, name)) for name, _ in _ffi.ShadowOcclusionCounters._fields_}
 
     def readback_objects(self, first_slot=0, n=None):
         n = self.capacity - first_slot if n is None else int(n)
```
